# Chenxu1103/UNET-

Measured on AMD Instinct MI355X. Metric: frames/sec 512x512 3-class UNet++ inference; mask vs CPU reference, higher is better.
Workload: dtype f16 (MFMA operands split hi+lo, 3 MFMAs per product, f32 accumulate); 1 GPU; UNet++ 3-class 512x512 batch=16/GPU fp16-MFMA on 1 MI355X, synthetic frames, f32 NCHW in HBM -> uint8 mask in HBM; arch=nested, precision=exact, frames_per_gpu=16, global_batch=16, micro_batch=16, parallelism=frame-sharded x1, weights replicated (RCCL bcast)

## Files before the change

### unet-_amd/csrc/conv3x3_mfma.h

```cpp
#pragma once
#include <hip/hip_runtime.h>
#include <stdint.h>

namespace unetpp {

typedef _Float16 half_t;
typedef __attribute__((ext_vector_type(8))) _Float16 half8;
typedef __attribute__((ext_vector_type(2))) _Float16 half2v;
typedef __attribute__((ext_vector_type(16))) float float16v;
typedef __attribute__((ext_vector_type(4))) unsigned int u32x4;

struct ConvArgs {
  const half_t* in0;
  const half_t* in1;
  const half_t* wpk;
  const float* scale;
  const float* bias;
  half_t* out;
  half_t* pool_out;
  int N, H, W, C0, C1, Cout;
  int tiles_x, tiles_y;
  int nct;
  int nchunks;
  int ksplit;
  float* kpart;
  unsigned* kcnt;
  int gdec[5];
  int pair9;
  const float* head_w;
  const float* head_b;
  int head_C;
  float* logits;
  uint8_t* mask;
  uint8_t* cable;
  uint8_t* tape;
  float* probs;
  int rule;
  float t_cable, t_tape, bg_margin, ct_margin;
  unsigned* status;
  const float* zinit;
  const void* raw_in;
  int raw_fmt;
  const half_t* c1w;
  const float* c1_scale;
  const float* c1_bias;
#ifdef UNETPP_WS_DBG
  int dbg;
  unsigned long long* stamps;
#endif
};

constexpr unsigned ST_OVERFLOW = 1u, ST_NAN = 2u;
constexpr float F16_MAX = 65504.0f;
__device__ __forceinline__ void range_flag(unsigned* status, bool out_of_range, bool is_nan) {
  const unsigned long long bn = __builtin_amdgcn_ballot_w64(is_nan);
  const unsigned long long bo = __builtin_amdgcn_ballot_w64(out_of_range && !is_nan);
  if ((threadIdx.x & 63) == 0 && status) atomicOr(status, (bn ? ST_NAN : 0u) | (bo ? ST_OVERFLOW : 0u));
}

__device__ __forceinline__ void apply_rule(int rule, float p0, float p1, float p2, float tc, float tt, float bgm,
                                           float ctm, bool& cable, bool& tape) {
  const int winner = (p1 > p0) ? ((p2 > p1) ? 2 : 1) : ((p2 > p0) ? 2 : 0);
  if (rule == 1) {
    cable = winner == 1 && p1 >= tc && (p1 - p0) >= bgm;
    tape = winner == 2 && p2 >= tt && (p2 - p0) >= bgm;
  } else if (rule == 2) {
    cable = winner == 1 && p1 >= tc && p0 <= bgm;
    tape = winner == 2 && p2 >= tt && p0 <= bgm;
  } else {
    const bool cand_c = p1 >= tc && p1 >= p0 + bgm;
    const bool cand_t = p2 >= tt && p2 >= p0 + bgm;
    cable = cand_c && p1 >= p2 + ctm;
    tape = cand_t && p2 >= p1 + ctm;
    if (cable && tape) { cable = p1 >= p2; tape = !cable; }
  }
}

template <int P, int KC, int NW, int MW, int WAVES, bool UPF = false>
struct ConvCfg {
  static constexpr int NT = WAVES * 64;
  static constexpr int TH = WAVES * MW, TW = 32, HALO_W = TW + 2, NHALO = (TH + 2) * HALO_W;
  static constexpr int KG = KC / 8, BN = 32 * NW;
  static constexpr int U = P * KG;
  static constexpr int PPP = 64 / U;
  static constexpr int HALO_PIECES = (NHALO + PPP - 1) / PPP;
  static constexpr int HALO_BYTES = HALO_PIECES * 1024;
  static constexpr int HALO_ITERS = (HALO_PIECES + WAVES - 1) / WAVES;
  static constexpr int SLAB_BYTES = P * 9 * KC * BN * 2;
  static constexpr int BUF_BYTES = HALO_BYTES + SLAB_BYTES;
  static constexpr int LSH = TH / 2 + 2, LSW = TW / 2 + 2, LS_PX = LSH * LSW;
  static constexpr int LS_REC = P * 32;
  static constexpr int LS_PIECES = (LS_PX * LS_REC + 1023) / 1024;
  static constexpr int LS_BYTES = UPF ? LS_PIECES * 1024 : 0;
  static constexpr int LS_ITERS = (LS_PIECES + WAVES - 1) / WAVES;
  static constexpr int LDS_BYTES = 2 * BUF_BYTES + 2 * LS_BYTES;
  static constexpr int SLAB_PIECES = SLAB_BYTES / 1024;
  static_assert(U == 2 || U == 4, "unit count per pixel");
  static_assert(SLAB_BYTES % 1024 == 0, "slab must be a whole number of 1 KiB DMA pieces");
  static_assert(LDS_BYTES <= 160 * 1024, "LDS budget");
};

__device__ __forceinline__ void split_f16(float v, half_t& hi, half_t& lo) {
  v = fminf(v, F16_MAX);
  hi = (half_t)v;
  lo = (half_t)(v - (float)hi);
}

typedef __attribute__((address_space(3))) char lds_char_t;

template <class Args>
__device__ __forceinline__ void touch_kernarg_lines() {
  const int* ka = (const int*)__builtin_amdgcn_kernarg_segment_ptr();
  int touched = 0;
#pragma unroll
  for (int o = 0; o < (int)(sizeof(Args) / 4); o += 16) touched |= ka[o];
  asm volatile("" :: "s"(touched));
}

__device__ __forceinline__ void glds16(const void* sbase, unsigned voff, unsigned lds_dst) {
  unsigned keep;
  asm volatile("s_mov_b32 %0, m0\n\ts_mov_b32 m0, %3\n\ts_nop 0\n\tglobal_load_lds_dwordx4 %1, %2\n\ts_mov_b32 m0, %0"
               : "=&s"(keep)
               : "v"(voff), "s"(sbase), "s"(lds_dst)
               : "memory");
}

template <bool NT = false>
__device__ __forceinline__ void blds16(__amdgpu_buffer_rsrc_t rsrc, unsigned voff, int soff, unsigned lds_dst) {
  unsigned keep;
  if (NT)
    asm volatile("s_mov_b32 %0, m0\n\ts_mov_b32 m0, %4\n\ts_nop 0\n\tbuffer_load_dwordx4 %1, %2, %3 offen nt lds\n\ts_mov_b32 m0, %0"
                 : "=&s"(keep)
                 : "v"(voff), "s"(rsrc), "s"(soff), "s"(lds_dst)
                 : "memory");
  else
    asm volatile("s_mov_b32 %0, m0\n\ts_mov_b32 m0, %4\n\ts_nop 0\n\tbuffer_load_dwordx4 %1, %2, %3 offen lds\n\ts_mov_b32 m0, %0"
                 : "=&s"(keep)
                 : "v"(voff), "s"(rsrc), "s"(soff), "s"(lds_dst)
                 : "memory");
}

__device__ __forceinline__ void split_pack2(float v0, float v1, unsigned& wh, unsigned& wl) {
  half2v ph = {(half_t)v0, (half_t)v1};
  wh = __builtin_bit_cast(unsigned, ph);
  unsigned l;
  asm("v_fma_mixlo_f16 %0, %1, -1.0, %2 op_sel_hi:[1,0,0]" : "=v"(l) : "v"(wh), "v"(v0));
  asm("v_fma_mixhi_f16 %0, %1, -1.0, %2 op_sel:[1,0,0] op_sel_hi:[1,0,0]" : "+v"(l) : "v"(wh), "v"(v1));
  wl = l;
}

typedef __attribute__((ext_vector_type(2))) short short2v;
constexpr float X8_LO_DIV = 0.00390625f, X8_X_DIV = 8.0f;
constexpr float X8_LO_MUL = 0.00390625f;
constexpr int X8_SCALE_W = 127 + 6, X8_SCALE_A = 127 - 8;
__device__ __forceinline__ void split_pack4_x8(float v0, float v1, float v2, float v3, unsigned& h0, unsigned& h1, unsigned& l8, unsigned& x8) {
  half2v p0 = {(half_t)v0, (half_t)v1}, p1 = {(half_t)v2, (half_t)v3};
  h0 = __builtin_bit_cast(unsigned, p0); h1 = __builtin_bit_cast(unsigned, p1);
  float l0, l1, l2, l3;
  asm("v_fma_mix_f32 %0, %1, -1.0, %2 op_sel_hi:[1,0,0]" : "=v"(l0) : "v"(h0), "v"(v0));
  asm("v_fma_mix_f32 %0, %1, -1.0, %2 op_sel:[1,0,0] op_sel_hi:[1,0,0]" : "=v"(l1) : "v"(h0), "v"(v1));
  asm("v_fma_mix_f32 %0, %1, -1.0, %2 op_sel_hi:[1,0,0]" : "=v"(l2) : "v"(h1), "v"(v2));
  asm("v_fma_mix_f32 %0, %1, -1.0, %2 op_sel:[1,0,0] op_sel_hi:[1,0,0]" : "=v"(l3) : "v"(h1), "v"(v3));
  short2v t = {0, 0};
  t = __builtin_amdgcn_cvt_scalef32_pk_bf8_f32(t, l0, l1, X8_LO_DIV, false);
  t = __builtin_amdgcn_cvt_scalef32_pk_bf8_f32(t, l2, l3, X8_LO_DIV, true);
  l8 = __builtin_bit_cast(unsigned, t);
  short2v u = {0, 0};
  u = __builtin_amdgcn_cvt_scalef32_pk_bf8_f32(u, v0, v1, X8_X_DIV, false);
  u = __builtin_amdgcn_cvt_scalef32_pk_bf8_f32(u, v2, v3, X8_X_DIV, true);
  x8 = __builtin_bit_cast(unsigned, u);
}

template <int P, bool X8 = false>
__device__ __forceinline__ void pack_store_octets(const float (&v)[16], half_t* dst, size_t blk_stride, bool ok, int h) {
  unsigned wh[4][2], wl[4][2];
  if (X8) {
#pragma unroll
    for (int q = 0; q < 4; ++q) split_pack4_x8(v[4 * q], v[4 * q + 1], v[4 * q + 2], v[4 * q + 3], wh[q][0], wh[q][1], wl[q][0], wl[q][1]);
  }
#pragma unroll
  for (int q = 0; q < 4; ++q)
#pragma unroll
    for (int w2 = 0; w2 < 2; ++w2) {
      const float v0 = v[4 * q + 2 * w2], v1 = v[4 * q + 2 * w2 + 1];
      if (X8) {
      } else if (P == 2) {
        split_pack2(v0, v1, wh[q][w2], wl[q][w2]);
      } else {
        half2v ph = {(half_t)v0, (half_t)v1};
        wh[q][w2] = __builtin_bit_cast(unsigned, ph);
      }
    }
#pragma unroll
  for (int pi = 0; pi < 2; ++pi) {
#pragma unroll
    for (int w2 = 0; w2 < 2; ++w2) {
      auto r = __builtin_amdgcn_permlane32_swap(wh[2 * pi][w2], wh[2 * pi + 1][w2], false, false);
      wh[2 * pi][w2] = r[0]; wh[2 * pi + 1][w2] = r[1];
      if (P == 2) {
        auto r2 = __builtin_amdgcn_permlane32_swap(wl[2 * pi][w2], wl[2 * pi + 1][w2], false, false);
        wl[2 * pi][w2] = r2[0]; wl[2 * pi + 1][w2] = r2[1];
      }
    }
    if (ok) {
      u32x4 o = {wh[2 * pi][0], wh[2 * pi][1], wh[2 * pi + 1][0], wh[2 * pi + 1][1]};
      *(u32x4*)(dst + pi * blk_stride + 8 * h) = o;
      if (P == 2) {
        u32x4 o2 = {wl[2 * pi][0], wl[2 * pi][1], wl[2 * pi + 1][0], wl[2 * pi + 1][1]};
        *(u32x4*)(dst + pi * blk_stride + 16 + 8 * h) = o2;
      }
    }
  }
}

template <int P, bool X8 = false>
__device__ __forceinline__ void pack_store_rows8(const float (&v)[16], half_t* dst, size_t blk_stride, bool ok, int h, bool dbg_nostore = false, bool dbg_coalesced = false) {
#pragma unroll
  for (int pi = 0; pi < 2; ++pi) {
    unsigned wh[4], wl[4];
    if (X8) {
      split_pack4_x8(v[8 * pi], v[8 * pi + 1], v[8 * pi + 2], v[8 * pi + 3], wh[0], wh[1], wl[0], wl[1]);
      split_pack4_x8(v[8 * pi + 4], v[8 * pi + 5], v[8 * pi + 6], v[8 * pi + 7], wh[2], wh[3], wl[2], wl[3]);
    }
#pragma unroll
    for (int i = 0; i < 4; ++i) {
      if (X8) {
      } else if (P == 2) {
        split_pack2(v[8 * pi + 2 * i], v[8 * pi + 2 * i + 1], wh[i], wl[i]);
      } else {
        half2v ph = {(half_t)v[8 * pi + 2 * i], (half_t)v[8 * pi + 2 * i + 1]};
        wh[i] = __builtin_bit_cast(unsigned, ph);
      }
    }
#ifdef UNETPP_WS_DBG
    if (dbg_nostore) {
      asm volatile("" :: "v"(wh[0]), "v"(wh[1]), "v"(wh[2]), "v"(wh[3]));
      if (P == 2) asm volatile("" :: "v"(wl[0]), "v"(wl[1]), "v"(wl[2]), "v"(wl[3]));
      continue;
    }
    if (dbg_coalesced) {
      const int lane_ = (int)(threadIdx.x & 63), p_ = lane_ & 31;
      half_t* row = dst - p_ * (P * 16) + pi * blk_stride;
      if (ok) {
        *(u32x4*)(row + lane_ * 8) = (u32x4){wh[0], wh[1], wh[2], wh[3]};
        if (P == 2) *(u32x4*)(row + 512 + lane_ * 8) = (u32x4){wl[0], wl[1], wl[2], wl[3]};
      }
      continue;
    }
#endif
    if (ok) {
      *(u32x4*)(dst + pi * blk_stride + 8 * h) = (u32x4){wh[0], wh[1], wh[2], wh[3]};
      if (P == 2) *(u32x4*)(dst + pi * blk_stride + 16 + 8 * h) = (u32x4){wl[0], wl[1], wl[2], wl[3]};
    }
  }
}

constexpr int HEAD_FUSED_MAX_CLASSES = 8;

template <int P, int KC, int NW, int MW, int WAVES, bool POOL, bool HEAD = false, bool UPF = false>
__global__ __launch_bounds__(WAVES * 64, 1)
void conv3x3_bias_relu_kernel(ConvArgs a) {
  touch_kernarg_lines<ConvArgs>();
  using C = ConvCfg<P, KC, NW, MW, WAVES, UPF>;
  static_assert(!UPF || (!POOL && !HEAD && KC == 16 && MW == 2), "fused upsample: plain 16-row tiles only");
  constexpr int NT = C::NT, TH = C::TH, TW = C::TW, HALO_W = C::HALO_W;
  constexpr int KG = C::KG, BN = C::BN, PPP = C::PPP;
  constexpr int ITERS = C::HALO_ITERS;
  extern __shared__ __attribute__((aligned(16))) char smem[];

  const int tid = threadIdx.x;
  const int lane = tid & 63;
  const int wave = __builtin_amdgcn_readfirstlane(tid >> 6);
  const int H = a.H, W = a.W;
  const int tiles_img = a.tiles_x * a.tiles_y;
  const int total_tiles = a.N * tiles_img * a.nct;
  const int nch0 = (a.C0 + KC - 1) / KC;
  const unsigned lds_base = (unsigned)(unsigned long)(lds_char_t*)smem;

  const int my_u = lane / PPP;
  const int my_pl = my_u / KG, my_k8 = (my_u % KG) * 8;
  int hyx[ITERS];
#pragma unroll
  for (int it = 0; it < ITERS; ++it) {
    const int hp = (wave + it * WAVES) * PPP + lane % PPP;
    const int hy = hp / HALO_W, hx = hp - hy * HALO_W;
    hyx[it] = (hp < C::NHALO) ? ((hy << 8) | hx) : -1;
  }

  constexpr unsigned OOB = 0x80000000u;
  unsigned voff0[ITERS], voff1[ITERS];
  __amdgpu_buffer_rsrc_t rsrc0, rsrc1;
  const char* wsrc;
  const unsigned img_bytes0 = (unsigned)(H * W * P * a.C0 * 2);
  const unsigned img_bytes1 = (unsigned)((UPF ? (H >> 1) * (W >> 1) : H * W) * P * a.C1 * 2);
  int cur_n, cur_y0, cur_x0, cur_ct;
  auto decode = [&](int t, int& n, int& y0, int& x0, int& ct) {
    ct = t % a.nct;
    int pt = t / a.nct;
    const int tx = pt % a.tiles_x; pt /= a.tiles_x;
    const int ty = pt % a.tiles_y;
    n = pt / a.tiles_y;
    x0 = tx * TW; y0 = ty * TH;
  };
  const int cb0 = a.C0 < 16 ? a.C0 : 16;
  const unsigned plane_bytes0 = (unsigned)(H * W * P * cb0 * 2);
  const int Hs = UPF ? (H >> 1) : H, Ws = UPF ? (W >> 1) : W;
  const unsigned plane_bytes1 = (unsigned)(Hs * Ws * P * 16 * 2);
  constexpr int UP_ITEMS = C::NHALO * KG;
  constexpr int UP_ROUNDS = UPF ? (UP_ITEMS + NT - 1) / NT : 0;
  constexpr int LSR = UPF ? C::LS_ITERS : 1, UPR = UPF ? UP_ROUNDS : 1;
  unsigned voffL[LSR];
  int up_o00[UPR], up_o01[UPR], up_o10[UPR];
  float up_lx1[UPR], up_ly0[UPR], up_ly1[UPR];
  int up_dst[UPR];
  const float up_sh = Hs > 1 ? (float)(Hs - 1) / (float)(H - 1) : 0.f;
  const float up_sw = Ws > 1 ? (float)(Ws - 1) / (float)(W - 1) : 0.f;
  if (UPF) {
#pragma unroll
    for (int r = 0; r < UPR; ++r) {
      const int i = tid + r * NT;
      const int kg = i / C::NHALO, hp = i - kg * C::NHALO;
      up_dst[r] = i < UP_ITEMS ? (hp / PPP) * 1024 + (kg * PPP + hp % PPP) * 16 : -1;
    }
  }
  auto setup_sources = [&](int n, int y0, int x0, int ct) {
#pragma unroll
    for (int it = 0; it < ITERS; ++it) {
      const int hy = hyx[it] >> 8, hx = hyx[it] & 255;
      const int gy = y0 + hy - 1, gx = x0 + hx - 1;
      const int pl = my_pl, k8 = my_k8;
      const bool ok = hyx[it] >= 0 && gy >= 0 && gy < H && gx >= 0 && gx < W;
      const unsigned pix = (unsigned)((gy * W + gx) * P + pl);
      voff0[it] = (ok && k8 < a.C0) ? (unsigned)(k8 >> 4) * plane_bytes0 + (pix * cb0 + (k8 & 15)) * 2u : OOB;
      voff1[it] = ok ? (unsigned)(k8 >> 4) * plane_bytes1 + (pix * 16 + (k8 & 15)) * 2u : OOB;
    }
    rsrc0 = __builtin_amdgcn_make_buffer_rsrc((void*)(a.in0 + (size_t)n * H * W * P * a.C0), 0, (int)img_bytes0, 0x00020000);
    rsrc1 = __builtin_amdgcn_make_buffer_rsrc((void*)(a.in1 ? a.in1 + (size_t)n * Hs * Ws * P * a.C1 : a.in0), 0,
                                              (int)(a.in1 ? img_bytes1 : 0u), 0x00020000);
    wsrc = (const char*)a.wpk + (size_t)ct * a.nchunks * C::SLAB_BYTES;
    if (UPF) {
      const int ybase = (int)(up_sh * (float)max(y0 - 1, 0)), xbase = (int)(up_sw * (float)max(x0 - 1, 0));
      constexpr int PXP = 1024 / C::LS_REC, PARTS = C::LS_REC / 16;
#pragma unroll
      for (int it = 0; it < LSR; ++it) {
        const int lp = (wave + it * WAVES) * PXP + lane / PARTS;
        const int ly = lp / C::LSW, lx = lp - ly * C::LSW;
        const int yy = min(ybase + ly, Hs - 1), xx = min(xbase + lx, Ws - 1);
        voffL[it] = lp < C::LS_PX ? (unsigned)((yy * Ws + xx) * C::LS_REC + (lane % PARTS) * 16) : OOB;
      }
#pragma unroll
      for (int r = 0; r < UPR; ++r) {
        const int i = tid + r * NT;
        const int kg = i / C::NHALO, hp = i - kg * C::NHALO;
        const int hy = hp / HALO_W, hx = hp - hy * HALO_W;
        const int gy = y0 + hy - 1, gx = x0 + hx - 1;
        const bool inside = i < UP_ITEMS && gy >= 0 && gy < H && gx >= 0 && gx < W;
        const float fy = up_sh * (float)max(gy, 0), fx = up_sw * (float)max(gx, 0);
        const int yy0 = min((int)fy, Hs - 1), xx0 = min((int)fx, Ws - 1);
        const int yy1 = yy0 + (yy0 < Hs - 1 ? 1 : 0), xx1 = xx0 + (xx0 < Ws - 1 ? 1 : 0);
        const float ly1 = fminf(fmaxf(fmaf(up_sh, (float)max(gy, 0), -(float)yy0), 0.f), 1.f);
        const float lx1 = fminf(fmaxf(fmaf(up_sw, (float)max(gx, 0), -(float)xx0), 0.f), 1.f);
        const int ry0 = min(max(yy0 - ybase, 0), C::LSH - 1), ry1 = min(max(yy1 - ybase, 0), C::LSH - 1);
        const int rx0 = min(max(xx0 - xbase, 0), C::LSW - 1), rx1 = min(max(xx1 - xbase, 0), C::LSW - 1);
        up_o00[r] = (ry0 * C::LSW + rx0) * C::LS_REC + kg * 16;
        up_o01[r] = (ry0 * C::LSW + rx1) * C::LS_REC + kg * 16;
        up_o10[r] = (ry1 * C::LSW + rx0) * C::LS_REC + kg * 16;
        up_lx1[r] = lx1;
        up_ly0[r] = inside ? 1.f - ly1 : 0.f;
        up_ly1[r] = inside ? ly1 : 0.f;
      }
    }
  };

  auto halo_dma_one = [&](int c, int halo_off, int it) {
    const int piece = wave + it * WAVES;
    if (C::HALO_PIECES % WAVES != 0 && piece >= C::HALO_PIECES) return;
    const unsigned dst = lds_base + halo_off + piece * 1024;
    if (c < nch0) blds16(rsrc0, voff0[it], c * (KC / 16) * (int)plane_bytes0, dst);
    else if (!UPF) blds16(rsrc1, voff1[it], (c - nch0) * (KC / 16) * (int)plane_bytes1, dst);
  };
  const int ls_base = 2 * C::BUF_BYTES;
  auto ls_dma_one = [&](int c, int it) {
    const int piece = wave + it * WAVES;
    if (C::LS_PIECES % WAVES != 0 && piece >= C::LS_PIECES) return;
    blds16(rsrc1, voffL[it], (c - nch0) * (int)plane_bytes1, lds_base + ls_base + (c & 1) * C::LS_BYTES + piece * 1024);
  };
  auto up_item = [&](int c, int halo_off, int r) {
    if (up_dst[r] < 0) return;
    const char* ls = smem + ls_base + (c & 1) * C::LS_BYTES;
    const int o11 = up_o10[r] + (up_o01[r] - up_o00[r]);
    const half8 h00 = *(const half8*)(ls + up_o00[r]), h01 = *(const half8*)(ls + up_o01[r]);
    const half8 h10 = *(const half8*)(ls + up_o10[r]), h11 = *(const half8*)(ls + o11);
    half8 l00, l01, l10, l11;
    if (P == 2) {
      l00 = *(const half8*)(ls + up_o00[r] + 32); l01 = *(const half8*)(ls + up_o01[r] + 32);
      l10 = *(const half8*)(ls + up_o10[r] + 32); l11 = *(const half8*)(ls + o11 + 32);
    }
    const float lx1 = up_lx1[r], lx0 = 1.f - lx1, ly0 = up_ly0[r], ly1 = up_ly1[r];
    half8 oh, ol;
#pragma unroll
    for (int e = 0; e < 8; ++e) {
      float t0, t1;
      if (P == 2) {
        t0 = fmaf(lx1, (float)l01[e], fmaf(lx1, (float)h01[e], fmaf(lx0, (float)l00[e], lx0 * (float)h00[e])));
        t1 = fmaf(lx1, (float)l11[e], fmaf(lx1, (float)h11[e], fmaf(lx0, (float)l10[e], lx0 * (float)h10[e])));
      } else {
        t0 = fmaf(lx1, (float)h01[e], lx0 * (float)h00[e]);
        t1 = fmaf(lx1, (float)h11[e], lx0 * (float)h10[e]);
      }
      const float v = fmaf(ly1, t1, ly0 * t0);
      const half_t hi = (half_t)v;
      oh[e] = hi;
      if (P == 2) ol[e] = (half_t)(v - (float)hi);
    }
    char* dst = smem + halo_off + up_dst[r];
    *(half8*)dst = oh;
    if (P == 2) *(half8*)(dst + KG * PPP * 16) = ol;
  };
  constexpr int DMA_PER_WAVE = (C::SLAB_PIECES + WAVES - 1) / WAVES;
  auto slab_dma_one = [&](int c, int slab_off, int p) {
    const int piece = wave + p * WAVES;
    if (C::SLAB_PIECES % WAVES == 0 || piece < C::SLAB_PIECES)
      glds16(wsrc + (size_t)c * C::SLAB_BYTES + piece * 1024, lane * 16, lds_base + slab_off + piece * 1024);
  };

  int a_off[MW + 2][3];
#pragma unroll
  for (int r = 0; r < MW + 2; ++r)
#pragma unroll
    for (int dx = 0; dx < 3; ++dx) {
      const int hp = (wave * MW + r) * HALO_W + (lane & 31) + dx;
      a_off[r][dx] = (hp / PPP) * 1024 + ((lane >> 5) * PPP + hp % PPP) * 16;
    }
  const int b_lane_off = ((lane >> 5) * BN + (lane & 31)) * 16;

  struct Frag { half8 ah[MW], al[MW], bh[NW], bl[NW]; };
  auto load_frags = [&](Frag& f, const char* halo, const char* slab, int step) {
    const int tap = step % 9, s = step / 9;
    const int dy = tap / 3, dx = tap % 3;
#pragma unroll
    for (int m = 0; m < MW; ++m) {
      const char* p = halo + a_off[m + dy][dx] + (2 * s) * PPP * 16;
// ... 233 lines not shown
```

### unet-_amd/csrc/conv3x3_ws.h

```cpp
#pragma once
#include "conv3x3_mfma.h"

namespace unetpp {

template <int P, bool UPF, bool C0F = false, int NW_ = 1, int MW_ = 4, bool X8_ = false>
struct WsCfg {
  static constexpr bool X8 = X8_;
  static_assert(!X8 || P == 2, "EXACT8 keeps the 64-byte pixel records of the two-plane format");
  static constexpr int NT = 512, NCONS = 4, NPROD = 4, MW = MW_, NW = NW_;
  static constexpr int TH = NCONS * MW, TW = 32, HALO_W = TW + 2, NHALO = (TH + 2) * HALO_W;
  static constexpr int KC = 16, KG = 2, BN = 32 * NW;
  static_assert(MW % 2 == 0 && NW * MW == 4, "108 MFMAs per chunk and consumer wave");
  static constexpr int U = P * KG, PPP = 64 / U;
  static constexpr int HALO_PIECES = (NHALO + PPP - 1) / PPP, HALO_BYTES = HALO_PIECES * 1024;
  static constexpr int HALO_ITERS = (HALO_PIECES + NPROD - 1) / NPROD;
  static constexpr int SLAB_MAIN = 9 * KC * BN * 2;
  static constexpr int SLAB_BYTES = X8 ? SLAB_MAIN + 5 * 2 * 2 * BN * 16 : P * SLAB_MAIN, SLAB_PIECES = SLAB_BYTES / 1024;
  static constexpr int SLAB_ITERS = (SLAB_PIECES + NPROD - 1) / NPROD;
  static constexpr int BUF_BYTES = HALO_BYTES + SLAB_BYTES;
  static constexpr int LSH = TH / 2 + 2, LSW = TW / 2 + 2, LS_PX = LSH * LSW, LS_REC = P * 32;
  static constexpr int LS_PIECES = (LS_PX * LS_REC + 1023) / 1024, LS_BYTES = UPF ? LS_PIECES * 1024 : 0;
  static constexpr int LS_ITERS = (LS_PIECES + NPROD - 1) / NPROD;
  static constexpr int PATCH_H = TH + 4, PATCH_W = TW + 4, PATCH_FLOATS = PATCH_H * PATCH_W * 3;
  static constexpr int PATCH_BYTES = C0F ? ((PATCH_FLOATS * 4 + 64 + 255) / 256) * 256 : 0;
  static constexpr int C0_GROUPS = (NHALO + 15) / 16, C0_ITERS = (C0_GROUPS + NPROD - 1) / NPROD;
  static constexpr bool HANDOFF = !UPF && !C0F;
  static constexpr int STG_WAVE = 2 * 16 * 64 * 4, STG_BYTES = HANDOFF ? NCONS * STG_WAVE : 0;
  static constexpr int LDS_BYTES = 2 * BUF_BYTES + 2 * LS_BYTES + 2 * PATCH_BYTES + STG_BYTES;
  static constexpr int BLK_Y = (TH + 2) / 2, BLK_X = HALO_W / 2, UP_ITEMS = BLK_Y * BLK_X * 4;
  static constexpr int UP_ROUNDS = (UP_ITEMS + NPROD * 64 - 1) / (NPROD * 64);
  static_assert(SLAB_BYTES % 1024 == 0 && LDS_BYTES <= 160 * 1024, "LDS budget");
};

typedef int int4v __attribute__((ext_vector_type(4)));
typedef int int8v __attribute__((ext_vector_type(8)));

__device__ __forceinline__ void lds_barrier() {
  __builtin_amdgcn_fence(__ATOMIC_RELEASE, "workgroup", "local");
  __builtin_amdgcn_s_barrier();
  __builtin_amdgcn_fence(__ATOMIC_ACQUIRE, "workgroup", "local");
}

template <int P, int ROWS, bool POOL, bool HEAD, bool X8 = false>
__device__ __forceinline__ void ws_epilogue(const ConvArgs& a, const float16v (&acc)[ROWS], const float2* sb_lds,
                                            const float* head_lds, int n, int gy0, int x0, int cbase, int lane) {
  const int H = a.H, W = a.W;
  const int h = lane >> 5;
  const int gx = x0 + (lane & 31);
  const int nbo = a.Cout >> 4;
  float v[ROWS][16];
  float vmax = 0.f;
#pragma unroll
  for (int r = 0; r < 16; ++r) {
    const int co = cbase + 16 * (r >> 3) + 8 * h + (r & 7);
    const float2 sb = sb_lds[co];
#pragma unroll
    for (int m = 0; m < ROWS; ++m) {
      v[m][r] = fmaxf(acc[m][r] * sb.x + sb.y, 0.f);
      if (!HEAD) vmax = fmaxf(vmax, v[m][r]);
    }
  }
  if (!HEAD && __builtin_amdgcn_ballot_w64(vmax > F16_MAX)) {
    range_flag(a.status, vmax > F16_MAX, false);
#pragma unroll
    for (int r = 0; r < 16; ++r)
#pragma unroll
      for (int m = 0; m < ROWS; ++m) v[m][r] = fminf(v[m][r], F16_MAX);
  }
  if (!HEAD) {
#pragma unroll
    for (int m = 0; m < ROWS; ++m) {
      const int gy = gy0 + m;
      const bool ok = gy < H && gx < W;
      const size_t blk = (size_t)H * W * P * 16;
      half_t* dst = a.out + ((size_t)n * nbo + (cbase >> 4)) * blk + ((size_t)gy * W + gx) * P * 16;
#ifdef UNETPP_WS_DBG
      pack_store_rows8<P, X8>(v[m], dst, blk, ok, h, (a.dbg & 262144) != 0, (a.dbg & 524288) != 0);
#else
      pack_store_rows8<P, X8>(v[m], dst, blk, ok, h);
#endif
    }
  } else {
    static_assert(!HEAD || ROWS % 2 == 0, "fused head: row pairs");
    const size_t hw = (size_t)H * W;
#pragma unroll
    for (int m2 = 0; m2 < ROWS / 2; ++m2) {
      float lg[HEAD_FUSED_MAX_CLASSES];
#pragma unroll
      for (int c = 0; c < HEAD_FUSED_MAX_CLASSES; ++c) {
        lg[c] = -INFINITY;
        if (c < a.head_C) {
          float wq[16];
#pragma unroll
          for (int q = 0; q < 4; ++q) {
            const float4 w4 = *(const float4*)(head_lds + c * 32 + 16 * (q >> 1) + 8 * h + 4 * (q & 1));
            wq[4 * q] = w4.x; wq[4 * q + 1] = w4.y; wq[4 * q + 2] = w4.z; wq[4 * q + 3] = w4.w;
          }
          const float bc = head_lds[a.head_C * 32 + c];
          float p0 = 0.f, p1 = 0.f;
#pragma unroll
          for (int r = 0; r < 16; ++r) { p0 = fmaf(v[2 * m2][r], wq[r], p0); p1 = fmaf(v[2 * m2 + 1][r], wq[r], p1); }
          auto sw = __builtin_amdgcn_permlane32_swap(__builtin_bit_cast(unsigned, p0), __builtin_bit_cast(unsigned, p1), false, false);
          unsigned s0 = sw[0], s1 = sw[1];
          asm volatile("s_nop 1" : "+v"(s0), "+v"(s1));
          lg[c] = bc + (__builtin_bit_cast(float, s0) + __builtin_bit_cast(float, s1));
        }
      }
      const int gy = gy0 + 2 * m2 + h;
      const bool ok = gy < H && gx < W;
      const size_t pix = (size_t)gy * W + gx;
      float best = lg[0];
      int besti = 0;
#pragma unroll
      for (int c = 1; c < HEAD_FUSED_MAX_CLASSES; ++c)
        if (lg[c] > best) { best = lg[c]; besti = c; }
      bool is_cable = besti == 1, is_tape = besti == 2;
      if (a.probs || a.rule) {
        float pe[HEAD_FUSED_MAX_CLASSES], sum = 0.f;
#pragma unroll
        for (int c = 0; c < HEAD_FUSED_MAX_CLASSES; ++c) {
          pe[c] = (c < a.head_C) ? expf(lg[c] - best) : 0.f;
          sum += pe[c];
        }
#pragma unroll
        for (int c = 0; c < HEAD_FUSED_MAX_CLASSES; ++c) {
          pe[c] = pe[c] / sum;
          if (ok && a.probs && c < a.head_C) a.probs[((size_t)n * a.head_C + c) * hw + pix] = pe[c];
        }
        if (a.rule) apply_rule(a.rule, pe[0], pe[1], pe[2], a.t_cable, a.t_tape, a.bg_margin, a.ct_margin, is_cable, is_tape);
      }
      if (ok) {
        if (a.logits) {
#pragma unroll
          for (int c = 0; c < HEAD_FUSED_MAX_CLASSES; ++c)
            if (c < a.head_C) a.logits[((size_t)n * a.head_C + c) * hw + pix] = lg[c];
        }
        const size_t o = (size_t)n * hw + pix;
        if (a.mask) a.mask[o] = (uint8_t)besti;
        if (a.cable) a.cable[o] = is_cable;
        if (a.tape) a.tape[o] = is_tape;
      }
    }
  }
  if (POOL) {
    static_assert(!POOL || ROWS % 2 == 0, "fused pool: row pairs");
    const int Hp = H >> 1, Wp = W >> 1;
#pragma unroll
    for (int m2 = 0; m2 < ROWS / 2; ++m2) {
      float pv[16];
#pragma unroll
      for (int r = 0; r < 16; ++r) {
        const float vm = fmaxf(v[2 * m2][r], v[2 * m2 + 1][r]);
        const float vn = __builtin_bit_cast(float, __builtin_amdgcn_mov_dpp(__builtin_bit_cast(int, vm), 0xB1, 0xF, 0xF, true));
        pv[r] = fmaxf(vm, vn);
      }
      const int py = (gy0 >> 1) + m2, px = (x0 >> 1) + ((lane & 31) >> 1);
      const bool ok = ((lane & 1) == 0) && py < Hp && px < Wp;
      const size_t blk = (size_t)Hp * Wp * P * 16;
      half_t* dst = a.pool_out + ((size_t)n * nbo + (cbase >> 4)) * blk + ((size_t)py * Wp + px) * P * 16;
#ifdef UNETPP_WS_DBG
      pack_store_rows8<P, X8>(pv, dst, blk, ok, h, (a.dbg & 262144) != 0);
#else
      pack_store_rows8<P, X8>(pv, dst, blk, ok, h);
#endif
    }
  }
}

template <int P, bool POOL, bool HEAD, bool UPF, bool C0F = false, int NW = 1, int MWP = 4, bool X8 = false, bool CAT2 = false>
__global__ __launch_bounds__(512, 2) void conv3x3_ws_kernel(ConvArgs a) {
  using C = WsCfg<P, UPF, C0F, NW, MWP, X8>;
  static_assert(!C0F || (!UPF && !HEAD && P == 2 && NW == 1), "fused first block: exact mode, no other fusion in the loader");
  static_assert(!HEAD || NW == 1, "the fused head needs all 32 channels of x0_4 in one 32-block");
  constexpr int NT = C::NT, MW = C::MW, TH = C::TH, TW = C::TW, HALO_W = C::HALO_W;
  constexpr int KC = C::KC, KG = C::KG, BN = C::BN, PPP = C::PPP;
  static_assert(!(POOL && HEAD) && !(UPF && (POOL || HEAD)), "one fused extra per kernel");
  static_assert(!CAT2 || (!UPF && !C0F && !POOL && !HEAD), "two full-resolution sources: the plain kernel only");
  extern __shared__ __attribute__((aligned(16))) char smem[];
#ifdef UNETPP_WS_DBG
  const unsigned long long rt_entry = __builtin_amdgcn_s_memrealtime();
#endif
  touch_kernarg_lines<ConvArgs>();

  const int tid = threadIdx.x;
  const int lane = tid & 63;
  const int wave = __builtin_amdgcn_readfirstlane(tid >> 6);
  const int H = a.H, W = a.W;
  const int tiles_img = a.tiles_x * a.tiles_y;
  const int KS = a.ksplit;
  const int total_tiles = a.N * tiles_img * a.nct * KS;
  const int nch0 = (a.C0 + KC - 1) / KC;
  const unsigned lds_base = (unsigned)(unsigned long)(lds_char_t*)smem;

  float2* sb_lds = (float2*)(smem + C::LDS_BYTES);
  float* head_lds = (float*)(smem + C::LDS_BYTES + a.Cout * 8);
  if (wave < C::NCONS) {
    for (int i = tid; i < a.Cout; i += C::NCONS * 64) sb_lds[i] = make_float2(a.scale[i], a.bias[i]);
    if (HEAD) {
      for (int i = tid; i < a.head_C * 32; i += C::NCONS * 64) head_lds[i] = a.head_w[i];
      for (int i = tid; i < a.head_C; i += C::NCONS * 64) head_lds[a.head_C * 32 + i] = a.head_b[i];
    }
  }

#ifdef UNETPP_WS_DBG
  const unsigned long long rt_staged = __builtin_amdgcn_s_memrealtime();
#endif
  const int G = (int)gridDim.x;
  const int slot = (G % 8 == 0) ? ((int)blockIdx.x % 8) * (G / 8) + (int)blockIdx.x / 8 : (int)blockIdx.x;
  int dec_ks = 0, dec_ct = 0, dec_tx = 0, dec_ty = 0, dec_n = 0, dec_t = -1;
  const int g_ks = a.gdec[0], g_ct = a.gdec[1], g_tx = a.gdec[2], g_ty = a.gdec[3], g_n = a.gdec[4];
  const bool small_radix = total_tiles < (1 << 22);
  auto divmod = [&](const int u, const int d, int& q, int& r) {
    int qq, rr;
    if (small_radix) {
      qq = (int)((float)u * __builtin_amdgcn_rcpf((float)d));
      rr = u - qq * d;
      const int up = rr >= d ? 1 : 0, dn = rr < 0 ? 1 : 0;
      qq += up - dn; rr += (dn - up) * d;
    } else {
      qq = u / d; rr = u - qq * d;
    }
    q = qq; r = rr;
  };
  auto decode = [&](int t, int& n, int& y0, int& x0) {
    if (t != dec_t) {
      if (dec_t >= 0 && t == dec_t + G) {
        dec_ks += g_ks;
        int carry = dec_ks >= KS ? 1 : 0;
        dec_ks -= carry ? KS : 0;
        dec_ct += g_ct + carry;
        carry = dec_ct >= a.nct ? 1 : 0;
        dec_ct -= carry ? a.nct : 0;
        dec_tx += g_tx + carry;
        carry = dec_tx >= a.tiles_x ? 1 : 0;
        dec_tx -= carry ? a.tiles_x : 0;
        dec_ty += g_ty + carry;
        carry = dec_ty >= a.tiles_y ? 1 : 0;
        dec_ty -= carry ? a.tiles_y : 0;
        dec_n += g_n + carry;
      } else {
        int u = t;
        divmod(u, KS, u, dec_ks);
        divmod(u, a.nct, u, dec_ct);
        divmod(u, a.tiles_x, u, dec_tx);
        divmod(u, a.tiles_y, dec_n, dec_ty);
      }
      dec_t = t;
    }
    n = dec_n; x0 = dec_tx * TW; y0 = dec_ty * TH;
  };
  if (slot >= total_tiles) return;
  const bool handoff = C::HANDOFF && a.nchunks >= 2 && KS == 1;

  typedef __attribute__((ext_vector_type(4))) float float4v;
  const int plane_id = tid - C::NCONS * 64;
  constexpr int PATCH_ELEMS = C::PATCH_FLOATS, PATCH_LOADS = C0F ? (PATCH_ELEMS + C::NPROD * 64 - 1) / (C::NPROD * 64) : 1;
  const int patch_base = 2 * C::BUF_BYTES + 2 * C::LS_BYTES;
  int pe_rc[PATCH_LOADS], pe_idx[PATCH_LOADS];
  if (C0F) {
#pragma unroll
    for (int i = 0; i < PATCH_LOADS; ++i) {
      const int e = plane_id + i * (C::NPROD * 64);
      int row, col, cs, idx;
      if (a.raw_fmt == 0) {
        const int ch = e / (C::PATCH_H * C::PATCH_W), rem = e - ch * (C::PATCH_H * C::PATCH_W);
        row = rem / C::PATCH_W; col = rem - row * C::PATCH_W; cs = ch; idx = rem * 3 + ch;
      } else {
        row = e / (C::PATCH_W * 3); const int b = e - row * (C::PATCH_W * 3);
        col = b / 3; cs = b - col * 3; idx = (row * C::PATCH_W + col) * 3 + (2 - cs);
      }
      pe_rc[i] = (row << 16) | (col << 2) | cs;
      pe_idx[i] = (e < PATCH_ELEMS && plane_id >= 0) ? idx : -1;
    }
  }
  auto patch_fetch = [&](int n, int y0, int x0, float (&val)[PATCH_LOADS]) {
    const size_t img = (size_t)H * W * 3;
    const __amdgpu_buffer_rsrc_t rs = __builtin_amdgcn_make_buffer_rsrc(
        (void*)((const char*)a.raw_in + (size_t)n * img * (a.raw_fmt == 0 ? 4 : 1)), 0, (int)(img * (a.raw_fmt == 0 ? 4 : 1)), 0x00020000);
    bool beyond = false;
#pragma unroll
    for (int i = 0; i < PATCH_LOADS; ++i) {
      const int gy = y0 - 2 + (pe_rc[i] >> 16), gx = x0 - 2 + ((pe_rc[i] >> 2) & 0x3fff), cs = pe_rc[i] & 3;
      const bool ok = pe_idx[i] >= 0 && gy >= 0 && gy < H && gx >= 0 && gx < W;
      float v;
      if (a.raw_fmt == 0) {
        v = __builtin_bit_cast(float, __builtin_amdgcn_raw_buffer_load_b32(rs, ok ? ((cs * H + gy) * W + gx) * 4 : (int)0x80000000, 0, 0));
      } else {
        const unsigned char b8 = __builtin_amdgcn_raw_buffer_load_b8(rs, ok ? (gy * W + gx) * 3 + cs : (int)0x80000000, 0, 0);
        v = __fdiv_rn((float)b8, 255.0f);
      }
      beyond |= !(fabsf(v) <= F16_MAX);
      val[i] = v;
    }
    if (__builtin_amdgcn_ballot_w64(beyond)) {
      bool nan = false;
#pragma unroll
      for (int i = 0; i < PATCH_LOADS; ++i) { nan |= val[i] != val[i]; val[i] = __builtin_amdgcn_fmed3f(val[i], -F16_MAX, F16_MAX); }
      range_flag(a.status, beyond, nan);
    }
  };
  auto patch_store = [&](int buf, const float (&val)[PATCH_LOADS]) {
    unsigned* pd = (unsigned*)(smem + patch_base + buf * C::PATCH_BYTES);
#pragma unroll
    for (int i = 0; i < PATCH_LOADS; ++i)
      if (pe_idx[i] >= 0) {
        unsigned wh, wl;
        split_pack2(val[i], 0.f, wh, wl);
        pd[pe_idx[i]] = (wh & 0xffffu) | (wl << 16);
      }
  };
  if (C0F && wave >= C::NCONS) {
    constexpr int SL_IT = (2 * C::SLAB_PIECES + C::NPROD - 1) / C::NPROD;
#pragma unroll
    for (int it = 0; it < SL_IT; ++it) {
      const int piece = (wave - C::NCONS) + it * C::NPROD;
      if (piece < 2 * C::SLAB_PIECES) {
        const int c = piece / C::SLAB_PIECES, pc = piece - c * C::SLAB_PIECES;
        glds16((const char*)a.wpk + (size_t)c * C::SLAB_BYTES + pc * 1024, lane * 16,
               lds_base + c * C::BUF_BYTES + C::HALO_BYTES + pc * 1024);
      }
    }
    if (plane_id < 32) {
      *(float*)(smem + patch_base + PATCH_ELEMS * 4 + (plane_id & 15) * 4 + (plane_id >> 4) * C::PATCH_BYTES) = 0.f;
    }
    int n0, y00, x00;
    decode(slot, n0, y00, x00);
    float pv[PATCH_LOADS];
    patch_fetch(n0, y00, x00, pv);
    patch_store(0, pv);
    asm volatile("s_waitcnt vmcnt(0)" ::: "memory");
  }
  if (C0F) __syncthreads();

#ifdef UNETPP_WS_DBG
#define WS_STAMP(i) { const unsigned long long now_ = __builtin_readcyclecounter(); st_sum[i] += now_ - st_t; st_t = now_; \
                      if (ev_ptr && ev_ptr < ev_end) *ev_ptr++ = ((unsigned long long)(i) << 56) | __builtin_amdgcn_s_memrealtime(); }
#define WS_EVLOG(role) unsigned long long* ev_ptr = (a.stamps && (a.dbg & 131072) && lane == 0 && blockIdx.x < 1024) ? a.stamps + (size_t)1024 * 32 + ((size_t)blockIdx.x * 2 + (role)) * 64 : nullptr; \
                       unsigned long long* const ev_end = ev_ptr + 60; if (ev_ptr) *ev_ptr++ = (63ull << 56) | rt_entry;
#define WS_STAMP_IN(i) if (a.dbg & 32768) { __builtin_amdgcn_sched_barrier(0); asm volatile("s_waitcnt lgkmcnt(0)" ::: "memory"); WS_STAMP(i) __builtin_amdgcn_sched_barrier(0); }
#define WS_EVT(i) { if (ev_ptr && ev_ptr < ev_end) *ev_ptr++ = ((unsigned long long)(i) << 56) | __builtin_amdgcn_s_memrealtime(); }
#else
#define WS_STAMP(i) {}
#define WS_STAMP_IN(i) {}
#define WS_EVT(i) {}
#endif
  if (C0F && wave >= C::NCONS) {
    const int pw = wave - C::NCONS;
#ifdef UNETPP_WS_DBG
    unsigned long long st_sum[11] = {0, 0, 0, 0, 0, 0, 0, 0, 0, 0, 0};
    unsigned long long st_t = __builtin_readcyclecounter();
    WS_EVLOG(1)
    if (pw != 0) ev_ptr = nullptr;
#endif
#ifndef UNETPP_C0_PRIO
#define UNETPP_C0_PRIO 1
#endif
    if (UNETPP_C0_PRIO) __builtin_amdgcn_s_setprio(UNETPP_C0_PRIO);
    typedef __attribute__((ext_vector_type(4))) float f32x4;
    typedef __attribute__((ext_vector_type(2))) unsigned u32x2;
    const int pxl = lane & 15, kq = lane >> 4;
    half8 wa_h[2], wa_l[2];
#pragma unroll
    for (int c = 0; c < 2; ++c) {
      wa_h[c] = *(const half8*)(a.c1w + ((size_t)(c * 2 + 0) * 64 + lane) * 8);
      wa_l[c] = *(const half8*)(a.c1w + ((size_t)(c * 2 + 1) * 64 + lane) * 8);
    }
    float sc1[2][4], bi1[2][4];
#pragma unroll
    for (int c = 0; c < 2; ++c)
#pragma unroll
      for (int r = 0; r < 4; ++r) { sc1[c][r] = a.c1_scale[16 * c + 4 * kq + r]; bi1[c][r] = a.c1_bias[16 * c + 4 * kq + r]; }
    int koff[8];
#pragma unroll
    for (int i = 0; i < 8; ++i) {
      if (kq < 3) koff[i] = (kq * C::PATCH_W * 3 + i) * 4;
      else koff[i] = i < 3 ? (i * C::PATCH_W * 3 + 8) * 4 : -1;
    }
    int g = 0;
    for (int tile = slot; tile < total_tiles; tile += G) {
      int n, y0, x0;
      decode(tile, n, y0, x0);
      const int tbuf = (g >> 1) & 1;
      const char* patch = smem + patch_base + tbuf * C::PATCH_BYTES;
      const int zero_off = PATCH_ELEMS * 4;
#pragma unroll
      for (int c = 0; c < 2; ++c, ++g) {
        float pv[PATCH_LOADS];
        const int ntile = tile + G;
        const bool have_next = c == 0 && ntile < total_tiles;
        if (have_next) {
          int n2, y2, x2;
          decode(ntile, n2, y2, x2);
          patch_fetch(n2, y2, x2, pv);
        }
        WS_STAMP(0)
        char* himg = smem + c * C::BUF_BYTES;
        float vmax = 0.f;
#ifndef UNETPP_C0_GB
#define UNETPP_C0_GB 2
#endif
        constexpr int GB = UNETPP_C0_GB;
        static_assert(C::C0_ITERS % GB == 0, "group batches");
        const int dst_lane = ((kq >> 1) * PPP + pxl) * 16 + (kq & 1) * 8;
        auto groups = [&](auto interior_tag) {
          constexpr bool INTERIOR = decltype(interior_tag)::value;
          int hy = (pw * 16 + pxl) / HALO_W, hx = (pw * 16 + pxl) - hy * HALO_W;
#pragma nounroll
          for (int b0 = 0; b0 < C::C0_ITERS; b0 += GB) {
            unsigned bw[GB][8];
            int ghy[GB], ghx[GB];
#pragma unroll
            for (int k = 0; k < GB; ++k) {
              ghy[k] = hy; ghx[k] = hx;
              const int hyc = min(hy, TH + 1);
              const int pix_off = (hyc * C::PATCH_W + hx) * 12;
#pragma unroll
              for (int i = 0; i < 8; ++i) bw[k][i] = *(const unsigned*)(patch + (koff[i] >= 0 ? pix_off + koff[i] : zero_off + 4 * i));
              hy += 1; hx += 64 - HALO_W;
              if (hx >= HALO_W) { hx -= HALO_W; hy += 1; }
            }
            f32x4 acc[GB];
#pragma unroll
            for (int k = 0; k < GB; ++k) {
              unsigned bh[4], bl[4];
#pragma unroll
              for (int i = 0; i < 4; ++i) {
                bh[i] = __builtin_amdgcn_perm(bw[k][2 * i + 1], bw[k][2 * i], 0x05040100u);
                bl[i] = __builtin_amdgcn_perm(bw[k][2 * i + 1], bw[k][2 * i], 0x07060302u);
              }
              const half8 xh = __builtin_bit_cast(half8, (u32x4){bh[0], bh[1], bh[2], bh[3]});
              const half8 xl = __builtin_bit_cast(half8, (u32x4){bl[0], bl[1], bl[2], bl[3]});
              acc[k] = (f32x4){0.f, 0.f, 0.f, 0.f};
              acc[k] = __builtin_amdgcn_mfma_f32_16x16x32_f16(wa_h[c], xl, acc[k], 0, 0, 0);
              acc[k] = __builtin_amdgcn_mfma_f32_16x16x32_f16(wa_l[c], xh, acc[k], 0, 0, 0);
              acc[k] = __builtin_amdgcn_mfma_f32_16x16x32_f16(wa_h[c], xh, acc[k], 0, 0, 0);
            }
#pragma unroll
            for (int k = 0; k < GB; ++k) {
              const int gi = pw + (b0 + k) * C::NPROD;
              const bool valid = gi * 16 + pxl < C::NHALO;
              float v[4];
#pragma unroll
              for (int r = 0; r < 4; ++r) v[r] = acc[k][r] * sc1[c][r] + bi1[c][r];
              vmax = fmaxf(fmaxf(vmax, v[0]), v[1]); vmax = fmaxf(fmaxf(vmax, v[2]), v[3]);
#pragma unroll
              for (int r = 0; r < 4; ++r) v[r] = __builtin_amdgcn_fmed3f(v[r], 0.f, F16_MAX);
              if (!INTERIOR) {
                const int gy = y0 - 1 + ghy[k], gx = x0 - 1 + ghx[k];
                const bool inside = gy >= 0 && gy < H && gx >= 0 && gx < W;
#pragma unroll
                for (int r = 0; r < 4; ++r) v[r] = inside ? v[r] : 0.f;
              }
              unsigned oh0, oh1, ol0, ol1;
              if (X8) {
                split_pack4_x8(v[0], v[1], v[2], v[3], oh0, oh1, ol0, ol1);
              } else {
                split_pack2(v[0], v[1], oh0, ol0);
                split_pack2(v[2], v[3], oh1, ol1);
              }
              if (valid) {
                char* dst = himg + gi * 1024 + dst_lane;
                *(u32x2*)dst = (u32x2){oh0, oh1};
                *(u32x2*)(dst + KG * PPP * 16) = (u32x2){ol0, ol1};
              }
            }
          }
        };
        if (y0 >= 1 && y0 + TH < H && x0 >= 1 && x0 + TW < W) groups(std::true_type());
        else groups(std::false_type());
        if (__builtin_amdgcn_ballot_w64(vmax > F16_MAX)) range_flag(a.status, vmax > F16_MAX, false);
        WS_STAMP(1)
        if (have_next) patch_store(tbuf ^ 1, pv);
        WS_STAMP(2)
        lds_barrier();
        WS_STAMP(3)
      }
    }
#ifdef UNETPP_WS_DBG
    if (a.stamps && pw == 0 && lane == 0)
#pragma unroll
      for (int i = 0; i < 11; ++i) a.stamps[((size_t)blockIdx.x * 2 + 1) * 16 + i] = st_sum[i];
    if (a.stamps && pw == 0 && lane == 0) a.stamps[((size_t)blockIdx.x * 2 + 1) * 16 + 12] = __builtin_amdgcn_s_memrealtime();
#endif
    return;
  }

  if (wave >= C::NCONS) {
    const int pw = wave - C::NCONS;
#ifdef UNETPP_WS_DBG
    const unsigned long long rt_prod = __builtin_amdgcn_s_memrealtime();
    { const int pr = (a.dbg >> 10) & 3; if (pr == 1) __builtin_amdgcn_s_setprio(1); else if (pr == 2) __builtin_amdgcn_s_setprio(2); else if (pr == 3) __builtin_amdgcn_s_setprio(3); }
#endif
    constexpr unsigned OOB = 0x80000000u;
    constexpr int ITERS = C::HALO_ITERS;
    int my_u = lane / PPP;
#ifdef UNETPP_WS_DBG
    if (a.dbg & 16384) my_u = lane % C::U;
#endif
    const int my_pl = my_u / KG, my_k8 = (my_u % KG) * 8;
    int hyx[ITERS];
#pragma unroll
    for (int it = 0; it < ITERS; ++it) {
      int hp = (pw + it * C::NPROD) * PPP + lane % PPP;
#ifdef UNETPP_WS_DBG
      if (a.dbg & 16384) hp = (pw + it * C::NPROD) * PPP + lane / C::U;
#endif
      const int hy = hp / HALO_W, hx = hp - hy * HALO_W;
      hyx[it] = (hp < C::NHALO) ? ((hy << 8) | hx) : -1;
    }
    const int cb0 = a.C0 < 16 ? a.C0 : 16;
    const unsigned plane_bytes0 = (unsigned)H * (unsigned)W * (unsigned)(P * cb0 * 2);
    const unsigned img_bytes0 = (unsigned)H * (unsigned)W * (unsigned)(P * a.C0 * 2);
    const int Hs = H >> 1, Ws = W >> 1;
    const unsigned plane_bytes1 = (unsigned)Hs * (unsigned)Ws * (unsigned)(P * 16 * 2);
    const unsigned img_bytes1 = (unsigned)Hs * (unsigned)Ws * (unsigned)(P * a.C1 * 2);
    const float up_sh = Hs > 1 ? (float)(Hs - 1) / (float)(H - 1) : 0.f;
    const float up_sw = Ws > 1 ? (float)(Ws - 1) / (float)(W - 1) : 0.f;

    int lane_off0[ITERS];
#pragma unroll
    for (int it = 0; it < ITERS; ++it) {
      const int hy = hyx[it] >> 8, hx = hyx[it] & 255;
      const bool valid = hyx[it] >= 0 && my_k8 < a.C0;
      lane_off0[it] = valid ? (my_k8 >> 4) * (int)plane_bytes0 + ((((hy - 1) * W + (hx - 1)) * P + my_pl) * cb0 + (my_k8 & 15)) * 2 : (int)OOB;
    }
    unsigned voff0[ITERS];
    __amdgpu_buffer_rsrc_t rsrc0, rsrc1;
    constexpr int LSR = UPF ? C::LS_ITERS : 1, UPR = UPF ? C::UP_ROUNDS : 1;
    unsigned voffL[LSR];
    int up_o00[UPR], up_o01[UPR], up_o10[UPR];
    float up_wx[UPR][4], up_wy[UPR][4];
    int up_st[UPR][4];
    int rd_swap = (P == 2 && !X8 && (lane & 16)) ? 32 : 0;
#ifdef UNETPP_WS_DBG
    if (a.dbg & 32) rd_swap = 0;
#endif
    if (UPF) {
#pragma unroll
      for (int r = 0; r < UPR; ++r) {
        const int i = pw * 64 + lane + r * (C::NPROD * 64);
        const int q = i & 3, blk = i >> 2;
        const int by = blk / C::BLK_X, bx = blk - by * C::BLK_X;
        const int hp0 = (2 * by) * HALO_W + 2 * bx;
#pragma unroll
        for (int px = 0; px < 4; ++px) {
          const int hp = hp0 + (px >> 1) * HALO_W + ((px & 1) ^ ((q >> 1) & 1));
          up_st[r][px] = (hp / PPP) * 1024 + ((q >> 1) * PPP + hp % PPP) * 16 + (q & 1) * 8;
        }
        if (i >= C::UP_ITEMS) up_st[r][0] = -1;
      }
    }

    auto setup_tile = [&](int n, int y0, int x0) {
      if (y0 >= 1 && y0 + TH < H && x0 >= 1 && x0 + TW < W) {
        const unsigned origin = ((unsigned)y0 * (unsigned)W + (unsigned)x0) * (unsigned)(P * cb0 * 2);
#pragma unroll
        for (int it = 0; it < ITERS; ++it) voff0[it] = origin + (unsigned)lane_off0[it];
      } else {
#pragma unroll
        for (int it = 0; it < ITERS; ++it) {
          const int hy = hyx[it] >> 8, hx = hyx[it] & 255;
          const int gy = y0 + hy - 1, gx = x0 + hx - 1;
          const bool ok = hyx[it] >= 0 && gy >= 0 && gy < H && gx >= 0 && gx < W;
          const unsigned pix = (unsigned)((gy * W + gx) * P + my_pl);
          voff0[it] = (ok && my_k8 < a.C0) ? (unsigned)(my_k8 >> 4) * plane_bytes0 + (pix * cb0 + (my_k8 & 15)) * 2u : OOB;
        }
      }
      rsrc0 = __builtin_amdgcn_make_buffer_rsrc((void*)(a.in0 + (size_t)n * H * W * P * a.C0), 0, (int)img_bytes0, 0x00020000);
      if (CAT2)
        rsrc1 = __builtin_amdgcn_make_buffer_rsrc((void*)(a.in1 + (size_t)n * H * W * P * a.C1), 0, (int)((unsigned)H * (unsigned)W * (unsigned)(P * a.C1 * 2)), 0x00020000);
      if (UPF) {
        rsrc1 = __builtin_amdgcn_make_buffer_rsrc((void*)(a.in1 + (size_t)n * Hs * Ws * P * a.C1), 0, (int)img_bytes1, 0x00020000);
        const int ybase = (int)(up_sh * (float)max(y0 - 1, 0)), xbase = (int)(up_sw * (float)max(x0 - 1, 0));
        constexpr int PXP = 1024 / C::LS_REC, PARTS = C::LS_REC / 16;
#pragma unroll
        for (int it = 0; it < LSR; ++it) {
          const int lp = (pw + it * C::NPROD) * PXP + lane / PARTS;
          const int ly = lp / C::LSW, lx = lp - ly * C::LSW;
          const int yy = min(ybase + ly, Hs - 1), xx = min(xbase + lx, Ws - 1);
          voffL[it] = lp < C::LS_PX ? (unsigned)((yy * Ws + xx) * C::LS_REC + (lane % PARTS) * 16) : OOB;
        }
#pragma unroll
        for (int r = 0; r < UPR; ++r) {
          const int i = pw * 64 + lane + r * (C::NPROD * 64);
          const int q = i & 3, blk = i >> 2;
          const int by = blk / C::BLK_X, bx = blk - by * C::BLK_X;
          const int gyA = y0 + 2 * by - 1, gxA = x0 + 2 * bx - 1;
          const int gyR = (gyA + 1 < H) ? gyA + 1 : gyA, gxR = (gxA + 1 < W) ? gxA + 1 : gxA;
          const float fyR = up_sh * (float)max(gyR, 0), fxR = up_sw * (float)max(gxR, 0);
          const int yy0 = min((int)fyR, Hs - 1), xx0 = min((int)fxR, Ws - 1);
          const int yy1 = yy0 + (yy0 < Hs - 1 ? 1 : 0), xx1 = xx0 + (xx0 < Ws - 1 ? 1 : 0);
          const int ry0 = min(max(yy0 - ybase, 0), C::LSH - 1), ry1 = min(max(yy1 - ybase, 0), C::LSH - 1);
          const int rx0 = min(max(xx0 - xbase, 0), C::LSW - 1), rx1 = min(max(xx1 - xbase, 0), C::LSW - 1);
          up_o00[r] = (ry0 * C::LSW + rx0) * C::LS_REC + q * 8 + rd_swap;
          up_o01[r] = (ry0 * C::LSW + rx1) * C::LS_REC + q * 8 + rd_swap;
          up_o10[r] = (ry1 * C::LSW + rx0) * C::LS_REC + q * 8 + rd_swap;
          const int xs = (q >> 1) & 1;
#pragma unroll
          for (int k = 0; k < 2; ++k) {
            const int gy = gyA + k, gx = gxA + (k ^ xs);
            const bool iny = gy >= 0 && gy < H, inx = gx >= 0 && gx < W;
            const float ly1 = fminf(fmaxf(up_sh * (float)max(gy, 0) - (float)yy0, 0.f), 1.f);
            const float lx1 = fminf(fmaxf(up_sw * (float)max(gx, 0) - (float)xx0, 0.f), 1.f);
            up_wy[r][2 * k] = iny ? 1.f - ly1 : 0.f; up_wy[r][2 * k + 1] = iny ? ly1 : 0.f;
            up_wx[r][2 * k] = inx ? 1.f - lx1 : 0.f; up_wx[r][2 * k + 1] = inx ? lx1 : 0.f;
          }
        }
      }
    };

#ifdef UNETPP_WS_DBG
    unsigned long long st_sum[11] = {0, 0, 0, 0, 0, 0, 0, 0, 0, 0, 0};
    unsigned long long st_t = 0;
    WS_EVLOG(1)
    if (pw != 0) ev_ptr = nullptr;
    if (ev_ptr) { *ev_ptr++ = (48ull << 56) | rt_staged; *ev_ptr++ = (49ull << 56) | rt_prod; }
    WS_EVT(50)
#endif
    auto up_rounds = [&](int c, int halo_off) {
      typedef __attribute__((ext_vector_type(2))) unsigned u32x2;
      const char* ls = smem + 2 * C::BUF_BYTES + (c & 1) * C::LS_BYTES;
      u32x2 hq[UPR][4], lq[UPR][4];
#pragma unroll
      for (int r = 0; r < UPR; ++r) {
        const int o11 = up_o10[r] + (up_o01[r] - up_o00[r]);
        const int off[4] = {up_o00[r], up_o01[r], up_o10[r], o11};
#pragma unroll
        for (int k = 0; k < 4; ++k) {
#ifdef UNETPP_WS_DBG
          if (a.dbg & 512) { hq[r][k] = (u32x2){0x3c003c00u, 0x3c003c00u}; lq[r][k] = (u32x2){0u, 0u}; continue; }
#endif
          hq[r][k] = *(const u32x2*)(ls + off[k]);
          if (P == 2) lq[r][k] = *(const u32x2*)(ls + (off[k] ^ 32));
        }
      }
      __builtin_amdgcn_sched_barrier(0);
      WS_STAMP_IN(8)
#pragma unroll
      for (int r = 0; r < UPR; ++r) {
        float v[4][4];
#pragma unroll
        for (int e = 0; e < 4; ++e) {
          float cc[4];
#pragma unroll
          for (int k = 0; k < 4; ++k) {
            if (X8) {
              const unsigned lo16 = __builtin_bit_cast(unsigned, (e >> 1) ? __builtin_amdgcn_cvt_scalef32_pk_f16_bf8(lq[r][k][0], X8_LO_MUL, true)
                                                                        : __builtin_amdgcn_cvt_scalef32_pk_f16_bf8(lq[r][k][0], X8_LO_MUL, false));
              if (e & 1) asm("v_fma_mix_f32 %0, %1, 1.0, %2 op_sel:[1,0,1] op_sel_hi:[1,0,1]" : "=v"(cc[k]) : "v"(hq[r][k][e >> 1]), "v"(lo16));
              else asm("v_fma_mix_f32 %0, %1, 1.0, %2 op_sel_hi:[1,0,1]" : "=v"(cc[k]) : "v"(hq[r][k][e >> 1]), "v"(lo16));
            } else if (P == 2) {
              if (e & 1) asm("v_fma_mix_f32 %0, %1, 1.0, %2 op_sel:[1,0,1] op_sel_hi:[1,0,1]" : "=v"(cc[k]) : "v"(hq[r][k][e >> 1]), "v"(lq[r][k][e >> 1]));
              else asm("v_fma_mix_f32 %0, %1, 1.0, %2 op_sel_hi:[1,0,1]" : "=v"(cc[k]) : "v"(hq[r][k][e >> 1]), "v"(lq[r][k][e >> 1]));
            } else {
              const unsigned hw = hq[r][k][e >> 1];
              const half2v hv = __builtin_bit_cast(half2v, hw);
              cc[k] = (float)hv[e & 1];
            }
          }
#pragma unroll
          for (int kx = 0; kx < 2; ++kx) {
            const float t0 = fmaf(up_wx[r][2 * kx + 1], cc[1], up_wx[r][2 * kx] * cc[0]);
            const float t1 = fmaf(up_wx[r][2 * kx + 1], cc[3], up_wx[r][2 * kx] * cc[2]);
#pragma unroll
            for (int ky = 0; ky < 2; ++ky) v[2 * ky + kx][e] = fmaf(up_wy[r][2 * ky + 1], t1, up_wy[r][2 * ky] * t0);
          }
        }
        WS_STAMP_IN(9)
#ifdef UNETPP_WS_DBG
        if (a.dbg & 64) { if (v[0][0] == 12345.f && v[3][3] == 7.f && v[1][2] == 3.f && v[2][1] == 9.f) a.status[1] = 1; continue; }
#endif
        if (up_st[r][0] >= 0) {
#pragma unroll
          for (int ky = 0; ky < 2; ++ky)
#pragma unroll
            for (int kx = 0; kx < 2; ++kx) {
              const int px = 2 * ky + kx;
              unsigned h0, h1, l0 = 0, l1 = 0;
              if (X8) {
                split_pack4_x8(v[px][0], v[px][1], v[px][2], v[px][3], h0, h1, l0, l1);
              } else if (P == 2) {
                split_pack2(v[px][0], v[px][1], h0, l0);
                split_pack2(v[px][2], v[px][3], h1, l1);
              } else {
                half2v a0 = {(half_t)v[px][0], (half_t)v[px][1]}, a1 = {(half_t)v[px][2], (half_t)v[px][3]};
                h0 = __builtin_bit_cast(unsigned, a0); h1 = __builtin_bit_cast(unsigned, a1);
              }
              const u32x2 oh = {h0, h1}, ol = {l0, l1};
              char* dst = smem + halo_off + up_st[r][px];
              *(u32x2*)dst = oh;
              if (P == 2) *(u32x2*)(dst + KG * PPP * 16) = ol;
            }
        }
        WS_STAMP_IN(10)
      }
    };

    const int stg_base = 2 * C::BUF_BYTES + 2 * C::LS_BYTES + 2 * C::PATCH_BYTES;
    int hn = 0, hy0 = 0, hx0 = 0, hct = 0;
    bool have_handoff = false;
    auto handoff_epilogue = [&]() {
      const char* st = smem + stg_base + pw * C::STG_WAVE + lane * 16;
      float16v pair[2];
#pragma unroll
      for (int i = 0; i < 2; ++i)
#pragma unroll
        for (int q = 0; q < 4; ++q) {
          typedef __attribute__((ext_vector_type(4))) float f32x4;
          const f32x4 v4 = *(const f32x4*)(st + (i * 4 + q) * 1024);
          pair[i][4 * q] = v4[0]; pair[i][4 * q + 1] = v4[1]; pair[i][4 * q + 2] = v4[2]; pair[i][4 * q + 3] = v4[3];
        }
      const int gy0 = hy0 + pw * MW + (MW == 4 ? 2 : 0);
      const int cbase = hct * BN + (MW == 4 ? 0 : 32);
      ws_epilogue<P, 2, POOL, HEAD, X8>(a, pair, sb_lds, head_lds, hn, gy0, hx0, cbase, lane);
    };
    int g = 0;
    const bool slabs_stay = a.nchunks == 2 && a.nct == 1 && KS == 1;
    const int chunks_per_share = KS == 1 ? a.nchunks : a.nchunks / KS;
#ifdef UNETPP_WS_DBG
    st_t = __builtin_readcyclecounter();
#endif
    WS_EVT(51)
    for (int tile = slot; tile < total_tiles; tile += G) {
      int n, y0, x0;
      decode(tile, n, y0, x0);
      WS_EVT(52)
      const char* wsrc = (const char*)a.wpk + (size_t)dec_ct * a.nchunks * C::SLAB_BYTES;
      const int tile_ct = dec_ct;
      const int c_begin = dec_ks * chunks_per_share, c_end = c_begin + chunks_per_share;
      setup_tile(n, y0, x0);
      WS_STAMP(7)
      for (int c = c_begin; c < c_end; ++c, ++g) {
        const int buf = (g & 1) * C::BUF_BYTES;
#ifdef UNETPP_WS_DBG
        if (!(a.dbg & 2))
#endif
        if (c < nch0) {
#pragma unroll
          for (int it = 0; it < ITERS; ++it) {
            const int piece = pw + it * C::NPROD;
            if (C::HALO_PIECES % C::NPROD == 0 || piece < C::HALO_PIECES)
              blds16<true>(rsrc0, voff0[it], c * (int)plane_bytes0, lds_base + buf + piece * 1024);
          }
        } else if (CAT2) {
#pragma unroll
          for (int it = 0; it < ITERS; ++it) {
            const int piece = pw + it * C::NPROD;
            if (C::HALO_PIECES % C::NPROD == 0 || piece < C::HALO_PIECES)
              blds16<true>(rsrc1, voff0[it], (c - nch0) * (int)plane_bytes0, lds_base + buf + piece * 1024);
          }
        }
#ifdef UNETPP_WS_DBG
        if (!(a.dbg & 8))
#endif
        if (!(slabs_stay && g >= 2))
#pragma unroll
        for (int it = 0; it < C::SLAB_ITERS; ++it) {
          const int piece = pw + it * C::NPROD;
          if (C::SLAB_PIECES % C::NPROD == 0 || piece < C::SLAB_PIECES)
            glds16(wsrc + (size_t)c * C::SLAB_BYTES + piece * 1024, lane * 16, lds_base + buf + C::HALO_BYTES + piece * 1024);
        }
        if (!UPF) { WS_STAMP(0) }
        if (UPF) {
#ifdef UNETPP_WS_DBG
          if (!(a.dbg & 2))
#endif
          if (c + 1 < a.nchunks && c + 1 >= nch0) {
#pragma unroll
            for (int it = 0; it < LSR; ++it) {
              const int piece = pw + it * C::NPROD;
              if (C::LS_PIECES % C::NPROD == 0 || piece < C::LS_PIECES)
                blds16(rsrc1, voffL[it], (c + 1 - nch0) * (int)plane_bytes1,
                       lds_base + 2 * C::BUF_BYTES + ((c + 1) & 1) * C::LS_BYTES + piece * 1024);
            }
          }
          if (c >= nch0) { WS_STAMP(3) } else { WS_STAMP(0) }
#ifdef UNETPP_WS_DBG
          if (!(a.dbg & 1))
#endif
          if (c >= nch0) up_rounds(c, buf);
          if (c >= nch0) { WS_STAMP(4) } else { WS_STAMP(0) }
        }
#ifdef UNETPP_WS_DBG
        if (!(a.dbg & 128))
#endif
        if (handoff && c == 1 && have_handoff) handoff_epilogue();
        asm volatile("s_waitcnt vmcnt(0)" ::: "memory");
        if (UPF && c >= nch0) { WS_STAMP(5) } else { WS_STAMP(1) }
        lds_barrier();
        if (UPF && c >= nch0) { WS_STAMP(6) } else { WS_STAMP(2) }
      }
      hn = n; hy0 = y0; hx0 = x0; hct = tile_ct; have_handoff = true;
    }
    if (handoff) {
      lds_barrier();
      if (have_handoff) handoff_epilogue();
    }
#ifdef UNETPP_WS_DBG
    if (a.stamps && pw == 0 && lane == 0)
#pragma unroll
      for (int i = 0; i < 11; ++i) a.stamps[((size_t)blockIdx.x * 2 + 1) * 16 + i] = st_sum[i];
    if (a.stamps && pw == 0 && lane == 0) a.stamps[((size_t)blockIdx.x * 2 + 1) * 16 + 12] = __builtin_amdgcn_s_memrealtime();
#endif
    return;
  }

  const int cw = wave;
#ifdef UNETPP_WS_DBG
  { const int pr = (a.dbg >> 12) & 3; if (pr == 1) __builtin_amdgcn_s_setprio(1); else if (pr == 2) __builtin_amdgcn_s_setprio(2); else if (pr == 3) __builtin_amdgcn_s_setprio(3); }
#endif
  int a_off[MW + 2][3];
#pragma unroll
  for (int r = 0; r < MW + 2; ++r)
#pragma unroll
    for (int dx = 0; dx < 3; ++dx) {
      const int hp = (cw * MW + r) * HALO_W + (lane & 31) + dx;
      a_off[r][dx] = (hp / PPP) * 1024 + ((lane >> 5) * PPP + hp % PPP) * 16;
    }
  const int b_lane_off = ((lane >> 5) * BN + (lane & 31)) * 16;
  struct AFrag { half8 h[MW + 2], l[MW + 2]; };
  struct BFrag { half8 h[NW], l[NW]; };
  auto load_a = [&](AFrag& f, const char* halo, int dx) {
#pragma unroll
    for (int r = 0; r < MW + 2; ++r) {
      const char* p = halo + a_off[r][dx];
      f.h[r] = *(const half8*)p;
      if (P == 2) f.l[r] = *(const half8*)(p + KG * PPP * 16);
    }
  };
  auto load_a_part = [&](AFrag& f, const char* halo, int dx, int r0, int r1) {
#pragma unroll
    for (int r = 0; r < MW + 2; ++r)
      if (r >= r0 && r < r1) {
        const char* p = halo + a_off[r][dx];
        f.h[r] = *(const half8*)p;
        if (P == 2) f.l[r] = *(const half8*)(p + KG * PPP * 16);
      }
  };
  auto load_b = [&](BFrag& f, const char* slab, int tap) {
#pragma unroll
    for (int j = 0; j < NW; ++j) {
      const int off = b_lane_off + (tap * KG * BN + j * 32) * 16;
      f.h[j] = *(const half8*)(slab + off);
      if (P == 2) f.l[j] = *(const half8*)(slab + off + 9 * KC * BN * 2);
    }
  };
  float16v acc[MW][NW];
  auto run_mfma = [&](const AFrag& fa, const BFrag& fb, int dy) {
#pragma unroll
    for (int m = 0; m < MW; ++m)
#pragma unroll
      for (int j = 0; j < NW; ++j) {
        if (P == 2) {
          acc[m][j] = __builtin_amdgcn_mfma_f32_32x32x16_f16(fb.h[j], fa.l[m + dy], acc[m][j], 0, 0, 0);
          acc[m][j] = __builtin_amdgcn_mfma_f32_32x32x16_f16(fb.l[j], fa.h[m + dy], acc[m][j], 0, 0, 0);
        }
        acc[m][j] = __builtin_amdgcn_mfma_f32_32x32x16_f16(fb.h[j], fa.h[m + dy], acc[m][j], 0, 0, 0);
      }
  };
  auto run_mfma_first = [&](const AFrag& fa, const BFrag& fb) {
    const float16v zero = {0.f, 0.f, 0.f, 0.f, 0.f, 0.f, 0.f, 0.f, 0.f, 0.f, 0.f, 0.f, 0.f, 0.f, 0.f, 0.f};
#pragma unroll
    for (int m = 0; m < MW; ++m)
#pragma unroll
      for (int j = 0; j < NW; ++j) {
        if (P == 2) {
          acc[m][j] = __builtin_amdgcn_mfma_f32_32x32x16_f16(fb.h[j], fa.l[m], zero, 0, 0, 0);
          acc[m][j] = __builtin_amdgcn_mfma_f32_32x32x16_f16(fb.l[j], fa.h[m], acc[m][j], 0, 0, 0);
          acc[m][j] = __builtin_amdgcn_mfma_f32_32x32x16_f16(fb.h[j], fa.h[m], acc[m][j], 0, 0, 0);
        } else {
          acc[m][j] = __builtin_amdgcn_mfma_f32_32x32x16_f16(fb.h[j], fa.h[m], zero, 0, 0, 0);
        }
      }
  };

  int g = 0;
#ifdef UNETPP_WS_DBG
  unsigned long long st_sum[8] = {0, 0, 0, 0, 0, 0, 0, 0};
  unsigned long long st_t = __builtin_readcyclecounter();
  const unsigned long long rt_begin = __builtin_amdgcn_s_memrealtime();
  WS_EVLOG(0)
  if (cw != 0) ev_ptr = nullptr;
  if (ev_ptr) *ev_ptr++ = (62ull << 56) | rt_begin;
#endif
  for (int tile = slot; tile < total_tiles; tile += G) {
    int n, y0, x0;
    decode(tile, n, y0, x0);
    const int ct = dec_ct, ks = dec_ks;
    const int c_begin = ks * (a.nchunks / KS), c_end = c_begin + a.nchunks / KS;
#pragma unroll
    for (int m = 0; m < MW; ++m)
#pragma unroll
      for (int j = 0; j < NW; ++j) {
        if (a.zinit && ks == 0) {
          typedef __attribute__((ext_vector_type(4))) float f32x4;
          const int gy = y0 + cw * MW + m, gx = x0 + (lane & 31);
          const bool in = gy < H && gx < W;
          const float* zp = a.zinit + (((size_t)n * (a.Cout >> 5) + ((ct * BN + j * 32) >> 5)) * ((size_t)H * W) + (size_t)gy * W + gx) * 32 + 8 * (lane >> 5);
#pragma unroll
          for (int q = 0; q < 4; ++q) {
            f32x4 z4 = {0.f, 0.f, 0.f, 0.f};
            if (in) z4 = *(const f32x4*)(zp + 16 * (q >> 1) + 4 * (q & 1));
#pragma unroll
            for (int i = 0; i < 4; ++i) acc[m][j][4 * q + i] = z4[i];
          }
        }
      }
    const bool from_zero = a.zinit == nullptr || ks != 0;
    int4v x9[MW];
    if (X8) {
#pragma unroll
      for (int m = 0; m < MW; ++m) x9[m] = (int4v){0, 0, 0, 0};
    }
    WS_STAMP(3)
    for (int c = c_begin; c < c_end; ++c, ++g) {
      lds_barrier();
      WS_STAMP(0)
      const char* halo = smem + (g & 1) * C::BUF_BYTES;
      const char* slab = halo + C::HALO_BYTES;
#ifdef UNETPP_WS_DBG
      if (a.dbg & 16) continue;
#endif
      if constexpr (X8) {
        constexpr int R = MW + 2;
        const char* xslab = slab + C::SLAB_MAIN;
        struct BM { half8 w[NW]; };
        struct BX { int8v w[NW]; };
        auto load_h = [&](half8 (&f)[R], int dx, int r0, int r1) {
#pragma unroll
          for (int r = 0; r < R; ++r)
            if (r >= r0 && r < r1) f[r] = *(const half8*)(halo + a_off[r][dx]);
        };
        auto load_x = [&](int dxa, int ra, int dxb, int rb) {
          const int4v lo = *(const int4v*)(halo + a_off[ra][dxa] + KG * PPP * 16);
          const int4v hi = *(const int4v*)(halo + a_off[rb][dxb] + KG * PPP * 16);
          return __builtin_shufflevector(lo, hi, 0, 1, 2, 3, 4, 5, 6, 7);
        };
        auto load_bm = [&](BM& f, int tap) {
#pragma unroll
          for (int j = 0; j < NW; ++j) f.w[j] = *(const half8*)(slab + b_lane_off + (tap * KG * BN + j * 32) * 16);
        };
        auto load_bx = [&](BX& f, int pair) {
#pragma unroll
          for (int j = 0; j < NW; ++j) {
            const char* p = xslab + pair * (2 * 2 * BN * 16) + b_lane_off + j * 32 * 16;
            const int4v lo = *(const int4v*)p, hi = *(const int4v*)(p + 2 * BN * 16);
            f.w[j] = __builtin_shufflevector(lo, hi, 0, 1, 2, 3, 4, 5, 6, 7);
          }
        };
        auto main_step = [&](const BM& b, const half8 (&hf)[R], int dy, bool first) {
#ifdef UNETPP_WS_DBG
          if (a.dbg & 4) return;
#endif
          const float16v zero = {0.f, 0.f, 0.f, 0.f, 0.f, 0.f, 0.f, 0.f, 0.f, 0.f, 0.f, 0.f, 0.f, 0.f, 0.f, 0.f};
#pragma unroll
          for (int m = 0; m < MW; ++m)
#pragma unroll
            for (int j = 0; j < NW; ++j)
              acc[m][j] = __builtin_amdgcn_mfma_f32_32x32x16_f16(b.w[j], hf[m + dy], first ? zero : acc[m][j], 0, 0, 0);
        };
        auto cross_step = [&](const BX& b, const int8v (&x)[R], int r0) {
#ifdef UNETPP_WS_DBG
          if (a.dbg & (4 | 65536)) return;
#endif
#pragma unroll
          for (int m = 0; m < MW; ++m)
#pragma unroll
            for (int j = 0; j < NW; ++j)
              acc[m][j] = __builtin_amdgcn_mfma_scale_f32_32x32x64_f8f6f4(b.w[j], x[m + r0], acc[m][j], 0 , 1 ,
                                                                         0, X8_SCALE_W, 0, X8_SCALE_A);
        };
        half8 h0[R], h1[R];
        int8v xa[R];
        BM bm0, bm1;
        BX bx0, bx1;
        load_h(h0, 0, 0, R);
        load_bm(bm0, 0);
        const bool first = c == c_begin && from_zero;
#pragma unroll
        for (int dy = 0; dy < 3; ++dy) {
          BM& b = (dy & 1) ? bm1 : bm0;
          BM& bn = (dy & 1) ? bm0 : bm1;
          load_bm(bn, dy < 2 ? (dy + 1) * 3 : 1);
          load_h(h1, 1, 2 * dy, 2 * dy + 2);
          __builtin_amdgcn_sched_barrier(0);
          if (dy == 0 && first) main_step(b, h0, 0, true); else main_step(b, h0, dy, false);
          __builtin_amdgcn_sched_barrier(0);
        }
#pragma unroll
        for (int dy = 0; dy < 3; ++dy) {
          BM& b = ((3 + dy) & 1) ? bm1 : bm0;
          BM& bn = ((3 + dy) & 1) ? bm0 : bm1;
          if (dy < 2) load_bm(bn, (dy + 1) * 3 + 1); else load_bx(bx0, 0);
#pragma unroll
          for (int r = 2 * dy; r < 2 * dy + 2 && r < R; ++r) xa[r] = load_x(0, r, 1, r);
          __builtin_amdgcn_sched_barrier(0);
          main_step(b, h1, dy, false);
          __builtin_amdgcn_sched_barrier(0);
        }
#pragma unroll
        for (int pr = 0; pr < 3; ++pr) {
          BX& b = (pr & 1) ? bx1 : bx0;
          BX& bn = (pr & 1) ? bx0 : bx1;
          if (pr < 2) load_bx(bn, pr + 1); else load_bm(bm0, 2);
          load_h(h0, 2, 2 * pr, 2 * pr + 2);
          __builtin_amdgcn_sched_barrier(0);
          cross_step(b, xa, pr);
          __builtin_amdgcn_sched_barrier(0);
        }
#pragma unroll
        for (int dy = 0; dy < 3; ++dy) {
          BM& b = (dy & 1) ? bm1 : bm0;
          BM& bn = (dy & 1) ? bm0 : bm1;
          if (dy < 2) load_bm(bn, (dy + 1) * 3 + 2); else load_bx(bx1, 3);
#pragma unroll
          for (int r = 2 * dy; r < 2 * dy + 2 && r < R; ++r) xa[r] = load_x(2, r, 2, r + 1 < R ? r + 1 : r);
          __builtin_amdgcn_sched_barrier(0);
          main_step(b, h0, dy, false);
          __builtin_amdgcn_sched_barrier(0);
        }
        load_bx(bx0, 4);
        int4v cur[MW];
#pragma unroll
        for (int m = 0; m < MW; ++m) cur[m] = *(const int4v*)(halo + a_off[m + 2][2] + KG * PPP * 16);
        __builtin_amdgcn_sched_barrier(0);
        cross_step(bx1, xa, 0);
        __builtin_amdgcn_sched_barrier(0);
        if (!(a.pair9 && ((c - c_begin) & 1) == 0)) {
          int8v xq[R];
#pragma unroll
          for (int m = 0; m < MW; ++m) xq[m] = __builtin_shufflevector(x9[m], cur[m], 0, 1, 2, 3, 4, 5, 6, 7);
          cross_step(bx0, xq, 0);
        }
#pragma unroll
        for (int m = 0; m < MW; ++m) x9[m] = cur[m];
        __builtin_amdgcn_sched_barrier(0);
        WS_STAMP(1)
        continue;
      }
      AFrag fa0, fa1;
      BFrag fb0, fb1;
      load_a(fa0, halo, 0);
      load_b(fb0, slab, 0);
#pragma unroll
      for (int dx = 0; dx < 3; ++dx) {
        AFrag& fa = (dx & 1) ? fa1 : fa0;
        AFrag& fan = (dx & 1) ? fa0 : fa1;
#pragma unroll
        for (int dy = 0; dy < 3; ++dy) {
          const int step = dx * 3 + dy;
          BFrag& fb = (step & 1) ? fb1 : fb0;
          BFrag& fbn = (step & 1) ? fb0 : fb1;
          if (step + 1 < 9) {
            const int ndx = (step + 1) / 3, ndy = (step + 1) % 3;
            load_b(fbn, slab, ndy * 3 + ndx);
          }
          if (dx < 2) load_a_part(fan, halo, dx + 1, 2 * dy, 2 * dy + 2);
          __builtin_amdgcn_sched_barrier(0);
#ifdef UNETPP_WS_DBG
          if (!(a.dbg & 4))
#endif
          {
            if (step == 0 && c == c_begin && from_zero) run_mfma_first(fa, fb);
            else run_mfma(fa, fb, dy);
          }
          __builtin_amdgcn_sched_barrier(0);
        }
      }
      WS_STAMP(1)
    }
#ifdef UNETPP_WS_DBG
    if (a.dbg & 256) { if (acc[0][0][0] == 12345.f && acc[MW - 1][NW - 1][5] == 7.f) a.status[1] = 1; continue; }
#endif
    if (KS > 1) {
      typedef __attribute__((ext_vector_type(4))) float f32x4;
      const int tile_id = tile / KS;
      const int ntile = total_tiles / KS;
      constexpr int WAVE_BYTES = MW * NW * 16 * 64 * 4;
      const __amdgpu_buffer_rsrc_t prs = __builtin_amdgcn_make_buffer_rsrc((void*)a.kpart, 0, KS * ntile * C::NCONS * WAVE_BYTES, 0x00020000);
      const int mine = ((ks * ntile + tile_id) * C::NCONS + cw) * WAVE_BYTES + lane * 16;
#pragma unroll
      for (int m = 0; m < MW; ++m)
#pragma unroll
        for (int j = 0; j < NW; ++j)
#pragma unroll
          for (int q = 0; q < 4; ++q)
            __builtin_amdgcn_raw_buffer_store_b128(__builtin_bit_cast(u32x4, (f32x4){acc[m][j][4 * q], acc[m][j][4 * q + 1], acc[m][j][4 * q + 2], acc[m][j][4 * q + 3]}),
                                                   prs, mine + ((m * NW + j) * 4 + q) * 1024, 0, 16 );
      asm volatile("s_waitcnt vmcnt(0)" ::: "memory");
      unsigned old = 0;
      if (lane == 0) old = __hip_atomic_fetch_add(a.kcnt + tile_id * C::NCONS + cw, 1u, __ATOMIC_RELAXED, __HIP_MEMORY_SCOPE_AGENT);
      old = __builtin_amdgcn_readfirstlane(old);
      if (old != (unsigned)(KS - 1)) { WS_STAMP(2) continue; }
      __builtin_amdgcn_fence(__ATOMIC_ACQUIRE, "wavefront");
      if (lane == 0) __hip_atomic_store(a.kcnt + tile_id * C::NCONS + cw, 0u, __ATOMIC_RELAXED, __HIP_MEMORY_SCOPE_AGENT);
      constexpr int HALF = MW * NW * 2;
      auto fetch = [&](f32x4 (&pv)[HALF], int u) {
        const int src = (((u >> 1) * ntile + tile_id) * C::NCONS + cw) * WAVE_BYTES + lane * 16 + (u & 1) * HALF * 1024;
#pragma unroll
        for (int t = 0; t < HALF; ++t) pv[t] = __builtin_bit_cast(f32x4, __builtin_amdgcn_raw_buffer_load_b128(prs, src + t * 1024, 0, 16 ));
      };
      auto add = [&](const f32x4 (&pv)[HALF], int u) {
#pragma unroll
        for (int m = 0; m < MW; ++m)
#pragma unroll
          for (int j = 0; j < NW; ++j)
#pragma unroll
            for (int q = 0; q < 4; ++q) {
              const int t = (m * NW + j) * 4 + q;
              if ((t >= HALF) != ((u & 1) != 0)) continue;
#pragma unroll
              for (int i = 0; i < 4; ++i) acc[m][j][4 * q + i] = u < 2 ? pv[t % HALF][i] : acc[m][j][4 * q + i] + pv[t % HALF][i];
            }
      };
      f32x4 pa[HALF], pb[HALF];
      fetch(pa, 0);
      for (int u = 0; u < 2 * KS; u += 2) {
        fetch(pb, u + 1);
        add(pa, u);
        if (u + 2 < 2 * KS) fetch(pa, u + 2);
        add(pb, u + 1);
      }
    }
#pragma unroll
    for (int m2 = 0; m2 < MW / 2; ++m2)
#pragma unroll
      for (int j = 0; j < NW; ++j) {
        const bool give = handoff && (MW == 4 ? m2 == 1 : j == 1);
        if (give) {
          char* st = smem + (2 * C::BUF_BYTES + 2 * C::LS_BYTES + 2 * C::PATCH_BYTES) + cw * C::STG_WAVE + lane * 16;
#pragma unroll
          for (int i = 0; i < 2; ++i)
#pragma unroll
            for (int q = 0; q < 4; ++q) {
              typedef __attribute__((ext_vector_type(4))) float f32x4;
              const float16v& v = acc[2 * m2 + i][j];
              *(f32x4*)(st + (i * 4 + q) * 1024) = (f32x4){v[4 * q], v[4 * q + 1], v[4 * q + 2], v[4 * q + 3]};
            }
        } else {
          const float16v pair[2] = {acc[2 * m2][j], acc[2 * m2 + 1][j]};
          ws_epilogue<P, 2, POOL, HEAD, X8>(a, pair, sb_lds, head_lds, n, y0 + cw * MW + 2 * m2, x0, ct * BN + j * 32, lane);
        }
      }
    WS_STAMP(2)
  }
  if (handoff) lds_barrier();
#ifdef UNETPP_WS_DBG
  if (a.stamps && cw == 0 && lane == 0)
#pragma unroll
    for (int i = 0; i < 4; ++i) a.stamps[((size_t)blockIdx.x * 2) * 16 + i] = st_sum[i];
  if (a.stamps && cw == 0 && lane == 0) {
    a.stamps[((size_t)blockIdx.x * 2) * 16 + 4] = rt_begin;
    a.stamps[((size_t)blockIdx.x * 2) * 16 + 6] = rt_entry;
    a.stamps[((size_t)blockIdx.x * 2) * 16 + 5] = __builtin_amdgcn_s_memrealtime();
  }
#endif
}
#undef WS_STAMP

}
```

### unet-_amd/csrc/unetpp_abi.hip

```cpp
#include <hip/hip_runtime.h>

#include <algorithm>
#include <cmath>
#include <cstdarg>
#include <cstdio>
#include <cstdlib>
#include <cstring>
#include <string>
#include <map>
#include <mutex>
#include <set>
#include <tuple>
#include <utility>
#include <vector>

#include "abi_common.h"
#include "aux_kernels.h"
#include "conv3x3_mfma.h"
#include "conv3x3_ws.h"
#include "convt2x2_mfma.h"
#include "tapmm_ws.h"

using namespace unetpp;

namespace {

thread_local std::string g_create_error;

constexpr uint32_t BLOB_MAGIC = 0x50504e55u;
constexpr uint32_t DS_BLOB_MAGIC = 0x53444e55u;
constexpr int BLOB_VERSION = 1;
const int NB[5] = {32, 64, 128, 256, 512};
const int SB[4] = {64, 128, 256, 512};

struct Tensor {
  std::string name;
  size_t off = 0;
  int C = 0;
  int lvl = 0;
  bool virt = false;
};

struct ConvLayer {
  std::string name;
  int cin_real = 0;
  int cout = 0;
  int lvl = 0;
  int in = -1, in2 = -1, out = -1, pool = -1;
  bool do_pool = false;
  int zt = -1;
  int y_t = -1, low_t = -1;
  half_t* tapw = nullptr;
  bool c0f = false;
  bool upf = false;
  bool ws = false;
  size_t w_off = 0, b_off = 0;
  int KC = 16, NW = 1, MW = 2, WAVES = 8;
  int nchunks = 1;
  half_t* wpk = nullptr;
  float* scale = nullptr;
  float* mult = nullptr;
};

struct ConvTLayer {
  std::string name;
  int cin = 0, cout = 0, lvl = 0;
  int in = -1, out = -1;
  size_t w_off = 0, b_off = 0;
  half_t* wpk = nullptr;
  float* scale = nullptr;
  float* mult = nullptr;
};

enum OpKind { OP_CONVERT, OP_CONV, OP_UP, OP_CONVT, OP_HEAD, OP_TAPMM, OP_UPSUM, OP_DS };
struct Op {
  OpKind kind;
  int idx = -1;
  int out = -1;
  bool fuse_head = false;
};

struct ProfRec {
  std::string name;
  double flops = 0, bytes = 0;
  int ev0 = -1, ev1 = -1;
};

}

struct unetpp_engine : unetpp_engine_common {
  int P = 2;
  bool x8 = false;
  int mb = 1;
  int num_cus = 256;
  char* arena = nullptr;
  size_t arena_bytes = 0;
  float* blob = nullptr;
  size_t blob_floats = 0;
  bool weights_loaded = false;
  std::vector<Tensor> tensors;
  std::vector<ConvLayer> convs;
  std::vector<ConvTLayer> convts;
  std::vector<Op> ops;
  int n_blob_layers = 0;
  int t_in8 = -1, t_head_in = -1;
  int head_cx = 32;
  size_t head_w_off = 0, head_b_off = 0;
  bool prof_on = false;
  std::vector<ProfRec> prof;
  int prof_used = 0;
  std::vector<hipEvent_t> evpool;
  int ev_used = 0;
  int prof_prev_ev = -1;
  hipStream_t prof_prev_stream = nullptr;
  int last_b = 0, last_h = 0, last_w = 0;
  bool keep_all = false;
  int nstreams = 1;
  size_t act_bytes = 0;
  size_t last_slot_off = 0;
  hipStream_t streams[4] = {nullptr, nullptr, nullptr, nullptr};
  hipEvent_t ev_start = nullptr, ev_done[4] = {nullptr, nullptr, nullptr, nullptr};
  half_t* c1w = nullptr;
  int c0f_conv1 = -1;
  unsigned* d_status = nullptr;
  int ksplit_max = 16, ksplit_min_chunks = 4, ksplit_gate = 4;
  int t_kpart = -1, t_kcnt = -1;
  bool kcnt_dirty = false;
  float* ds_w = nullptr;
  size_t ds_w_off[4] = {0, 0, 0, 0};
  float* ds_scratch[4] = {nullptr, nullptr, nullptr, nullptr};
  size_t ds_scr_off[4] = {0, 0, 0, 0};
  bool ds_loaded = false;
};

namespace unetpp {

unetpp_engine_common* unetpp_common(unetpp_engine* e) { return e; }

int fail(unetpp_engine* e, int code, const char* fmt, ...) {
  char buf[512];
  va_list ap;
  va_start(ap, fmt);
  vsnprintf(buf, sizeof buf, fmt, ap);
  va_end(ap);
  if (e) e->err = buf; else g_create_error = buf;
  return code;
}

hipError_t allow_full_lds(const void* kernel, int device, int bytes) {
  static std::mutex mu;
  static std::set<std::pair<int, const void*>> done;
  std::lock_guard<std::mutex> lock(mu);
  if (done.count({device, kernel})) return hipSuccess;
  hipError_t st = hipFuncSetAttribute(kernel, hipFuncAttributeMaxDynamicSharedMemorySize, bytes);
  if (st == hipSuccess) done.insert({device, kernel});
  return st;
}

}

namespace {

size_t blob_payload_floats(int arch, int C, int cin, int* n_layers = nullptr) {
  size_t n = 0;
  int layers = 0;
  if (arch == UNETPP_ARCH_NESTED) {
    int ci[9] = {cin, NB[0], NB[1], NB[2], NB[3], NB[3] + NB[4], NB[2] + NB[3], NB[1] + NB[2], NB[0] + NB[1]};
    int co[9] = {NB[0], NB[1], NB[2], NB[3], NB[4], NB[3], NB[2], NB[1], NB[0]};
    for (int b = 0; b < 9; ++b) {
      n += (size_t)co[b] * ci[b] * 9 + co[b];
      n += (size_t)co[b] * co[b] * 9 + co[b];
      layers += 2;
    }
    n += (size_t)C * NB[0] + C;
    layers += 1;
  } else {
    for (int l = 0; l < 4; ++l) {
      int ci = l == 0 ? cin : SB[l - 1];
      n += (size_t)SB[l] * ci * 9 + SB[l] + (size_t)SB[l] * SB[l] * 9 + SB[l];
      layers += 2;
    }
    for (int l = 2; l >= 0; --l) { n += (size_t)SB[l + 1] * SB[l] * 4 + SB[l]; layers += 1; }
    for (int l = 2; l >= 0; --l) {
      n += (size_t)SB[l] * (2 * SB[l]) * 9 + SB[l] + (size_t)SB[l] * SB[l] * 9 + SB[l];
      layers += 2;
    }
    n += (size_t)C * SB[0] + C;
    layers += 1;
  }
  if (n_layers) *n_layers = layers;
  return n;
}

struct LaunchCtx { int device; int num_cus; int ksplit_max = 1, ksplit_min_chunks = 4, ksplit_gate = 4; };

template <int P, int KC, int NW, int MW, int WAVES, bool POOL, bool HEAD, bool UPF = false>
hipError_t launch_conv_k(const LaunchCtx& cx, const ConvArgs& a, hipStream_t s) {
  using C = ConvCfg<P, KC, NW, MW, WAVES, UPF>;
  const int lds = C::LDS_BYTES + a.Cout * 8 + (HEAD ? ((a.head_C * 33 * 4 + 15) / 16) * 16 : 0);
  const int total = a.N * a.tiles_x * a.tiles_y * a.nct;
  const int per_cu = std::max(1, std::min(2, (160 * 1024) / lds));
  dim3 grid((unsigned)std::min(total, cx.num_cus * per_cu));
  auto k = conv3x3_bias_relu_kernel<P, KC, NW, MW, WAVES, POOL, HEAD, UPF>;
  hipError_t st = allow_full_lds((const void*)k, cx.device);
  if (st != hipSuccess) return st;
  hipLaunchKernelGGL(k, grid, dim3(C::NT), lds, s, a);
  return hipGetLastError();
}

template <int P, bool POOL, bool HEAD, bool UPF, bool C0F = false, int NW = 1, int MW = 4, bool X8 = false, bool CAT2 = false>
hipError_t launch_ws_k(const LaunchCtx& cx, ConvArgs a, hipStream_t s) {
  using C = WsCfg<P, UPF, C0F, NW, MW, X8>;
  a.tiles_x = (a.W + C::TW - 1) / C::TW; a.tiles_y = (a.H + C::TH - 1) / C::TH; a.nct = a.Cout / C::BN;
  const int lds = C::LDS_BYTES + a.Cout * 8 + (HEAD ? ((a.head_C * 33 * 4 + 15) / 16) * 16 : 0);
  const int tiles = a.N * a.tiles_x * a.tiles_y * a.nct;
  int ks = 1;
  if (!UPF && !C0F && !HEAD && a.kpart && a.kcnt && cx.ksplit_max > 1 && tiles * cx.ksplit_gate <= cx.num_cus)
    for (int d = 2; d <= cx.ksplit_max && tiles * d <= cx.num_cus && a.nchunks / d >= cx.ksplit_min_chunks; ++d)
      if (a.nchunks % d == 0 && !(a.pair9 && (a.nchunks / d) % 2)) ks = d;
  a.ksplit = ks;
  const int total = tiles * ks;
  dim3 grid((unsigned)std::min(total, cx.num_cus));
  {
    int t = (int)grid.x;
    a.gdec[0] = t % ks; t /= ks;
    a.gdec[1] = t % a.nct; t /= a.nct;
    a.gdec[2] = t % a.tiles_x; t /= a.tiles_x;
    a.gdec[3] = t % a.tiles_y;
    a.gdec[4] = t / a.tiles_y;
  }
  auto k = conv3x3_ws_kernel<P, POOL, HEAD, UPF, C0F, NW, MW, X8, CAT2>;
  hipError_t st = allow_full_lds((const void*)k, cx.device);
  if (st != hipSuccess) return st;
  hipLaunchKernelGGL(k, grid, dim3(C::NT), lds, s, a);
  return hipGetLastError();
}

template <bool X8>
hipError_t launch_ws_x(const LaunchCtx& cx, int P, const ConvArgs& a, bool pool, bool head, bool upf, bool c0f, hipStream_t s) {
  if (P != 2 || (upf && (pool || head)) || (pool && head)) return hipErrorInvalidValue;
  if (a.Cout >= 64 && a.Cout % 64 == 0) {
    if (head || c0f) return hipErrorInvalidValue;
    if (upf) return launch_ws_k<2, false, false, true, false, 2, 2, X8>(cx, a, s);
    if (pool) return a.in1 ? hipErrorInvalidValue : launch_ws_k<2, true, false, false, false, 2, 2, X8>(cx, a, s);
    if (a.in1) return launch_ws_k<2, false, false, false, false, 2, 2, X8, true>(cx, a, s);
    return launch_ws_k<2, false, false, false, false, 2, 2, X8>(cx, a, s);
  }
  if (a.in1 && !upf) return hipErrorInvalidValue;
  if (a.Cout != 32) return hipErrorInvalidValue;
  if (c0f) return (pool && !head && !upf && a.nchunks == 2) ? launch_ws_k<2, true, false, false, true, 1, 4, X8>(cx, a, s) : hipErrorInvalidValue;
  if (upf) return launch_ws_k<2, false, false, true, false, 1, 4, X8>(cx, a, s);
  if (head) return launch_ws_k<2, false, true, false, false, 1, 4, X8>(cx, a, s);
  if (pool) return launch_ws_k<2, true, false, false, false, 1, 4, X8>(cx, a, s);
  return launch_ws_k<2, false, false, false, false, 1, 4, X8>(cx, a, s);
}

hipError_t launch_ws(const LaunchCtx& cx, int P, bool x8, const ConvArgs& a, bool pool, bool head, bool upf, bool c0f, hipStream_t s) {
  return x8 ? launch_ws_x<true>(cx, P, a, pool, head, upf, c0f, s) : launch_ws_x<false>(cx, P, a, pool, head, upf, c0f, s);
}

template <int P, int KC, int NW, int MW, int WAVES>
hipError_t launch_conv_cfg(const LaunchCtx& cx, const ConvArgs& a, bool pool, bool head, bool upf, hipStream_t s) {
  if (a.zinit) return hipErrorInvalidValue;
  if constexpr (P == 2) {
    if (pool || head || upf) return hipErrorInvalidValue;
  } else {
    if constexpr (NW == 1 && MW == 2 && KC == 16) {
      if (upf) return (pool || head) ? hipErrorInvalidValue : launch_conv_k<P, KC, NW, MW, WAVES, false, false, true>(cx, a, s);
    }
    if (upf) return hipErrorInvalidValue;
    if constexpr (NW == 1) {
      if (head) return launch_conv_k<P, KC, NW, MW, WAVES, false, true>(cx, a, s);
    }
    if constexpr (MW == 2) {
      if (pool) return launch_conv_k<P, KC, NW, MW, WAVES, true, false>(cx, a, s);
    }
    if (pool) return hipErrorInvalidValue;
  }
  return launch_conv_k<P, KC, NW, MW, WAVES, false, false>(cx, a, s);
}

hipError_t launch_conv(const LaunchCtx& cx, int P, const ConvLayer& L, int mw, const ConvArgs& a, bool head, hipStream_t s) {
#define CASE(p, kc, nw, mw_, wv) \
  if (P == p && L.KC == kc && L.NW == nw && mw == mw_ && L.WAVES == wv) return launch_conv_cfg<p, kc, nw, mw_, wv>(cx, a, L.do_pool, head, L.upf, s);
  CASE(1, 16, 1, 2, 8)
  CASE(1, 32, 2, 2, 8)
  CASE(1, 16, 2, 2, 8)
  CASE(1, 16, 4, 2, 8)
  CASE(2, 16, 2, 2, 8)
  CASE(1, 16, 2, 1, 8)
  CASE(1, 32, 2, 1, 8)
  CASE(1, 16, 4, 1, 8)
  CASE(2, 16, 2, 1, 8)
#undef CASE
  return hipErrorInvalidValue;
}

int small_grid_rows(const ConvLayer& L, int num_cus, int nb, int H, int W, bool head) {
  if (L.do_pool || head || L.upf || L.zt >= 0 || L.NW == 1 || L.MW != 2) return L.MW;
  const int tiles = nb * ((W + 31) / 32) * ((H + 15) / 16) * (L.cout / (32 * L.NW));
  return tiles < num_cus ? 1 : L.MW;
}

void choose_cfg(int P, int cin_tensor, ConvLayer& L) {
  L.MW = 2; L.WAVES = 8;
  if (P == 1) {
    if (L.cout == 32) { L.NW = 1; L.KC = 16; }
    else if (L.cout == 64) { L.NW = 2; L.KC = (cin_tensor <= 16) ? 16 : 32; }
    else { L.NW = 4; L.KC = 16; }
  } else {
    L.KC = 16;
    L.NW = (L.cout == 32) ? 1 : 2;
  }
}

struct Launcher {
  unetpp_engine* e;
  hipStream_t s;
  int rc = UNETPP_OK;
  template <class F>
  void run(const std::string& name, double flops, double bytes, F&& f) {
    if (rc) return;
    ProfRec* r = nullptr;
    auto new_event = [&]() {
      if ((size_t)e->ev_used >= e->evpool.size()) {
        hipEvent_t ev = nullptr;
        hipError_t es = hipEventCreate(&ev);
        if (es != hipSuccess) { rc = fail(e, UNETPP_E_HIP, "hipEventCreate: %s", hipGetErrorString(es)); return -1; }
        e->evpool.push_back(ev);
      }
      return e->ev_used++;
    };
    if (e->prof_on) {
      if ((size_t)e->prof_used >= e->prof.size()) e->prof.push_back(ProfRec());
      r = &e->prof[e->prof_used++];
      r->name = name; r->flops = flops; r->bytes = bytes;
      if (e->prof_prev_ev >= 0 && e->prof_prev_stream == s) {
        r->ev0 = e->prof_prev_ev;
      } else {
        r->ev0 = new_event();
        if (r->ev0 < 0) { --e->prof_used; return; }
        (void)hipEventRecord(e->evpool[r->ev0], s);
      }
    }
    hipError_t st = f();
    if (st == hipSuccess) st = hipGetLastError();
    if (r) {
      r->ev1 = new_event();
      if (r->ev1 < 0) { --e->prof_used; e->prof_prev_ev = -1; return; }
      (void)hipEventRecord(e->evpool[r->ev1], s);
      e->prof_prev_ev = r->ev1; e->prof_prev_stream = s;
    }
    if (st != hipSuccess) rc = fail(e, UNETPP_E_HIP, "launch %s: %s", name.c_str(), hipGetErrorString(st));
  }
};

struct Builder {
  unetpp_engine* e;
  size_t act = 0;
  size_t off = 0;
  int tensor(const std::string& name, int C, int lvl, bool virt = false) {
    Tensor t;
    t.name = name; t.C = C; t.lvl = lvl; t.off = act; t.virt = virt;
    const unetpp_config& c = e->cfg;
    size_t px = (size_t)e->mb * (c.max_h >> lvl) * (c.max_w >> lvl);
    if (!virt) act += align_up(px * e->P * C * sizeof(half_t), 256);
    e->tensors.push_back(t);
    return (int)e->tensors.size() - 1;
  }
  int tensor_raw(const std::string& name, size_t bytes_per_px, int lvl) {
    Tensor t;
    t.name = name; t.C = 0; t.lvl = lvl; t.off = act;
    const unetpp_config& c = e->cfg;
    size_t px = (size_t)e->mb * (c.max_h >> lvl) * (c.max_w >> lvl);
    act += align_up(px * bytes_per_px, 256);
    e->tensors.push_back(t);
    return (int)e->tensors.size() - 1;
  }
  int conv(const std::string& name, int cin_real, int in, int in2, int out, bool pool_to = false, int pool = -1, bool emit_op = true) {
    ConvLayer L;
    L.name = name; L.cin_real = cin_real; L.in = in; L.in2 = in2; L.out = out; L.pool = pool; L.do_pool = pool_to;
    L.cout = e->tensors[out].C; L.lvl = e->tensors[out].lvl;
    L.w_off = off; off += (size_t)L.cout * cin_real * 9;
    L.b_off = off; off += L.cout;
    const int c0 = e->tensors[in].C, c1 = in2 >= 0 ? e->tensors[in2].C : 0;
    choose_cfg(e->P, c0 + c1, L);
    L.nchunks = (c0 + L.KC - 1) / L.KC + c1 / L.KC;
    e->convs.push_back(L);
    Op op; op.kind = OP_CONV; op.idx = (int)e->convs.size() - 1;
    if (emit_op) e->ops.push_back(op);
    return op.idx;
  }
  void convt(const std::string& name, int in, int out) {
    ConvTLayer T;
    T.name = name; T.in = in; T.out = out; T.cin = e->tensors[in].C; T.cout = e->tensors[out].C; T.lvl = e->tensors[in].lvl;
    T.w_off = off; off += (size_t)T.cin * T.cout * 4;
    T.b_off = off; off += T.cout;
    e->convts.push_back(T);
    Op op; op.kind = OP_CONVT; op.idx = (int)e->convts.size() - 1;
    e->ops.push_back(op);
  }
  void up(int src, int dst) { Op op; op.kind = OP_UP; op.idx = src; op.out = dst; e->ops.push_back(op); }
  void ds(int k, int node) { Op op; op.kind = OP_DS; op.idx = k; op.out = node; e->ops.push_back(op); }
  void head(int in, int cx) {
    e->t_head_in = in; e->head_cx = cx;
    e->head_w_off = off; off += (size_t)e->cfg.num_classes * cx;
    e->head_b_off = off; off += e->cfg.num_classes;
    Op op; op.kind = OP_HEAD; op.out = in; e->ops.push_back(op);
  }
};

void build_nested(unetpp_engine* e, Builder& b) {
  const bool c0f = e->P == 2;
  if (!c0f) { Op cv; cv.kind = OP_CONVERT; e->ops.push_back(cv); }
  e->t_in8 = b.tensor("in8", 8, 0, c0f);
  int x[5], xa[5], pooled[4], up[4], d[4], da[4];
  for (int l = 0; l < 5; ++l) {
    char nm[32];
    snprintf(nm, sizeof nm, "x%d_0", l);
    xa[l] = b.tensor(std::string(nm) + "a", NB[l], l, c0f && l == 0);
    x[l] = b.tensor(nm, NB[l], l);
    if (l < 4) pooled[l] = b.tensor(std::string(nm) + "p", NB[l], l + 1);
    snprintf(nm, sizeof nm, "conv%d_0", l);
    const int c1 = b.conv(std::string(nm) + ".conv1", l == 0 ? 3 : NB[l - 1], l == 0 ? e->t_in8 : pooled[l - 1], -1, xa[l], false, -1,
                          !(c0f && l == 0));
    const int c2 = b.conv(std::string(nm) + ".conv2", NB[l], xa[l], -1, x[l], l < 4, l < 4 ? pooled[l] : -1);
    if (c0f && l == 0) { e->convs[c2].c0f = true; e->c0f_conv1 = c1; }
  }
  for (int l = 3; l >= 0; --l) {
    char nm[32], tn[32];
    snprintf(tn, sizeof tn, "x%d_%d", l, 4 - l);
    const int low = l == 3 ? x[4] : d[l + 1];
    const char* tl = getenv("UNETPP_TAPMM");
    const bool tapmm = e->P == 2 && l >= 1 && (9 * NB[l]) % TapmmCfg::TN == 0 && strchr(tl ? tl : "23", '0' + l) != nullptr;
    if (tapmm) {
      snprintf(nm, sizeof nm, "conv%d_%d", l, 4 - l);
      const int yt = b.tensor_raw(std::string(tn) + "y", (size_t)9 * NB[l] * 4, l + 1);
      const int zt = b.tensor_raw(std::string(tn) + "z", (size_t)NB[l] * 4, l);
      da[l] = b.tensor(std::string(tn) + "a", NB[l], l);
      d[l] = b.tensor(tn, NB[l], l);
      { Op op; op.kind = OP_TAPMM; op.idx = (int)e->convs.size(); e->ops.push_back(op); }
      { Op op; op.kind = OP_UPSUM; op.idx = (int)e->convs.size(); e->ops.push_back(op); }
      const int ci = b.conv(std::string(nm) + ".conv1", NB[l] + NB[l + 1], x[l], -1, da[l]);
      ConvLayer& L = e->convs[ci];
      L.zt = zt; L.y_t = yt; L.low_t = low;
      L.nchunks = NB[l] / L.KC;
      b.conv(std::string(nm) + ".conv2", NB[l], da[l], -1, d[l]);
      b.ds(l, d[l]);
      continue;
    }
    const bool upf = e->P == 2 || l == 0;
    if (!upf) up[l] = b.tensor(std::string(tn) + "u", NB[l + 1], l);
    da[l] = b.tensor(std::string(tn) + "a", NB[l], l);
    d[l] = b.tensor(tn, NB[l], l);
    if (!upf) b.up(low, up[l]);
    snprintf(nm, sizeof nm, "conv%d_%d", l, 4 - l);
    const int ci = b.conv(std::string(nm) + ".conv1", NB[l] + NB[l + 1], x[l], upf ? low : up[l], da[l]);
    e->convs[ci].upf = upf;
    b.conv(std::string(nm) + ".conv2", NB[l], da[l], -1, d[l]);
    if (l == 0) e->ops.back().fuse_head = true;
    else b.ds(l, d[l]);
  }
  b.head(d[0], NB[0]);
}

void build_simple(unetpp_engine* e, Builder& b) {
  Op cv; cv.kind = OP_CONVERT; e->ops.push_back(cv);
  e->t_in8 = b.tensor("in8", 8, 0);
  int enc[4], enca[4], pooled[3];
  for (int l = 0; l < 4; ++l) {
    char nm[32];
    snprintf(nm, sizeof nm, "enc%d", l + 1);
    enca[l] = b.tensor(std::string(nm) + "a", SB[l], l);
    enc[l] = b.tensor(nm, SB[l], l);
    if (l < 3) pooled[l] = b.tensor(std::string(nm) + "p", SB[l], l + 1);
    b.conv(std::string(nm) + ".0", l == 0 ? 3 : SB[l - 1], l == 0 ? e->t_in8 : pooled[l - 1], -1, enca[l]);
    b.conv(std::string(nm) + ".2", SB[l], enca[l], -1, enc[l], l < 3, l < 3 ? pooled[l] : -1);
  }
  size_t up_w[3], up_b[3], dec_w[3][2], dec_b[3][2];
  size_t off = b.off;
  for (int l = 2; l >= 0; --l) { up_w[l] = off; off += (size_t)SB[l + 1] * SB[l] * 4; up_b[l] = off; off += SB[l]; }
  for (int l = 2; l >= 0; --l) {
    dec_w[l][0] = off; off += (size_t)SB[l] * 2 * SB[l] * 9; dec_b[l][0] = off; off += SB[l];
    dec_w[l][1] = off; off += (size_t)SB[l] * SB[l] * 9; dec_b[l][1] = off; off += SB[l];
  }
  int prev = enc[3];
  for (int l = 2; l >= 0; --l) {
    char nm[32];
    snprintf(nm, sizeof nm, "up%d", l + 1);
    int u = b.tensor(std::string(nm) + "t", SB[l], l);
    b.convt(nm, prev, u);
    e->convts.back().w_off = up_w[l]; e->convts.back().b_off = up_b[l];
    snprintf(nm, sizeof nm, "dec%d", l + 1);
    int da = b.tensor(std::string(nm) + "a", SB[l], l);
    int d = b.tensor(nm, SB[l], l);
    int c1 = b.conv(std::string(nm) + ".0", 2 * SB[l], u, enc[l], da);
    e->convs[c1].w_off = dec_w[l][0]; e->convs[c1].b_off = dec_b[l][0];
    int c2 = b.conv(std::string(nm) + ".2", SB[l], da, -1, d);
    e->convs[c2].w_off = dec_w[l][1]; e->convs[c2].b_off = dec_b[l][1];
    prev = d;
  }
  b.off = off;
  b.head(prev, SB[0]);
}

}

extern "C" {

#ifndef UNETPP_SRC_HASH
#define UNETPP_SRC_HASH "unknown"
#endif
#ifdef UNETPP_WS_DBG
#define UNETPP_BUILD_TAG " +wsdbg"
#else
#define UNETPP_BUILD_TAG ""
#endif
const char* unetpp_version(void) { return "unetpp-hip 0.3.0 (gfx950) src:" UNETPP_SRC_HASH UNETPP_BUILD_TAG; }

const char* unetpp_last_error(const unetpp_engine* e) { return e ? e->err.c_str() : g_create_error.c_str(); }

size_t unetpp_weights_blob_bytes(int num_classes, int in_channels) {
  return 32 + 4 * blob_payload_floats(UNETPP_ARCH_NESTED, num_classes, in_channels);
}

size_t unetpp_weights_blob_bytes_arch(int arch, int num_classes, int in_channels) {
  if (arch != UNETPP_ARCH_NESTED && arch != UNETPP_ARCH_SIMPLE) return 0;
  return 32 + 4 * blob_payload_floats(arch, num_classes, in_channels);
}

int unetpp_create(const unetpp_config* cfg, unetpp_engine** out) {
  if (!cfg || !out) return fail(nullptr, UNETPP_E_INVALID, "null argument");
  *out = nullptr;
  if (cfg->arch != UNETPP_ARCH_NESTED && cfg->arch != UNETPP_ARCH_SIMPLE) return fail(nullptr, UNETPP_E_INVALID, "arch=%d unknown", cfg->arch);
// ... 735 lines not shown
```

Measured before the change: 3999 frames/s.

## Read conv kernel args via kernarg pointer and split out split-K kernel variant

After: 4054 frames/s (median of 6 runs). 1.4% higher.

```diff
diff --git a/unet-_amd/csrc/conv3x3_mfma.h b/unet-_amd/csrc/conv3x3_mfma.h
--- a/unet-_amd/csrc/conv3x3_mfma.h
+++ b/unet-_amd/csrc/conv3x3_mfma.h
@@ -117,6 +117,18 @@
   asm volatile("" :: "s"(touched));
 }
 
+template <class Args>
+using KernArgs = const __attribute__((address_space(4))) Args*;
+template <class Args>
+__device__ __forceinline__ KernArgs<Args> kernargs_again(KernArgs<Args> p) {
+  asm volatile("" : "+s"(p));
+  return p;
+}
+template <class Args>
+__device__ __forceinline__ KernArgs<Args> kernargs() {
+  return kernargs_again<Args>((KernArgs<Args>)__builtin_amdgcn_kernarg_segment_ptr());
+}
+
 __device__ __forceinline__ void glds16(const void* sbase, unsigned voff, unsigned lds_dst) {
   unsigned keep;
   asm volatile("s_mov_b32 %0, m0\n\ts_mov_b32 m0, %3\n\ts_nop 0\n\tglobal_load_lds_dwordx4 %1, %2\n\ts_mov_b32 m0, %0"
@@ -138,6 +150,25 @@
                  : "=&s"(keep)
                  : "v"(voff), "s"(rsrc), "s"(soff), "s"(lds_dst)
                  : "memory");
+}
+
+__device__ __forceinline__ unsigned m0_run_begin() {
+  unsigned keep;
+  asm volatile("s_mov_b32 %0, m0" : "=s"(keep) :: "memory");
+  return keep;
+}
+__device__ __forceinline__ void m0_run_end(unsigned keep) {
+  asm volatile("s_mov_b32 m0, %0" :: "s"(keep) : "memory");
+}
+__device__ __forceinline__ void glds16_run(const void* sbase, unsigned voff, unsigned lds_dst) {
+  asm volatile("s_mov_b32 m0, %2\n\ts_nop 0\n\tglobal_load_lds_dwordx4 %0, %1" :: "v"(voff), "s"(sbase), "s"(lds_dst) : "memory");
+}
+template <bool NT = false>
+__device__ __forceinline__ void blds16_run(__amdgpu_buffer_rsrc_t rsrc, unsigned voff, int soff, unsigned lds_dst) {
+  if (NT)
+    asm volatile("s_mov_b32 m0, %3\n\ts_nop 0\n\tbuffer_load_dwordx4 %0, %1, %2 offen nt lds" :: "v"(voff), "s"(rsrc), "s"(soff), "s"(lds_dst) : "memory");
+  else
+    asm volatile("s_mov_b32 m0, %3\n\ts_nop 0\n\tbuffer_load_dwordx4 %0, %1, %2 offen lds" :: "v"(voff), "s"(rsrc), "s"(soff), "s"(lds_dst) : "memory");
 }
 
 __device__ __forceinline__ void split_pack2(float v0, float v1, unsigned& wh, unsigned& wl) {
diff --git a/unet-_amd/csrc/conv3x3_ws.h b/unet-_amd/csrc/conv3x3_ws.h
--- a/unet-_amd/csrc/conv3x3_ws.h
+++ b/unet-_amd/csrc/conv3x3_ws.h
@@ -41,13 +41,19 @@
   __builtin_amdgcn_fence(__ATOMIC_ACQUIRE, "workgroup", "local");
 }
 
+template <class T>
+__device__ __forceinline__ T opaque(T v) {
+  asm volatile("" : "+s"(v));
+  return v;
+}
+
 template <int P, int ROWS, bool POOL, bool HEAD, bool X8 = false>
-__device__ __forceinline__ void ws_epilogue(const ConvArgs& a, const float16v (&acc)[ROWS], const float2* sb_lds,
+__device__ __forceinline__ void ws_epilogue(KernArgs<ConvArgs> a, const float16v (&acc)[ROWS], const float2* sb_lds,
                                             const float* head_lds, int n, int gy0, int x0, int cbase, int lane) {
-  const int H = a.H, W = a.W;
+  const int H = a->H, W = a->W;
   const int h = lane >> 5;
   const int gx = x0 + (lane & 31);
-  const int nbo = a.Cout >> 4;
+  const int nbo = a->Cout >> 4;
   float v[ROWS][16];
   float vmax = 0.f;
 #pragma unroll
@@ -61,7 +67,7 @@
     }
   }
   if (!HEAD && __builtin_amdgcn_ballot_w64(vmax > F16_MAX)) {
-    range_flag(a.status, vmax > F16_MAX, false);
+    range_flag(a->status, vmax > F16_MAX, false);
 #pragma unroll
     for (int r = 0; r < 16; ++r)
 #pragma unroll
@@ -73,9 +79,9 @@
       const int gy = gy0 + m;
       const bool ok = gy < H && gx < W;
       const size_t blk = (size_t)H * W * P * 16;
-      half_t* dst = a.out + ((size_t)n * nbo + (cbase >> 4)) * blk + ((size_t)gy * W + gx) * P * 16;
-#ifdef UNETPP_WS_DBG
-      pack_store_rows8<P, X8>(v[m], dst, blk, ok, h, (a.dbg & 262144) != 0, (a.dbg & 524288) != 0);
+      half_t* dst = a->out + ((size_t)n * nbo + (cbase >> 4)) * blk + ((size_t)gy * W + gx) * P * 16;
+#ifdef UNETPP_WS_DBG
+      pack_store_rows8<P, X8>(v[m], dst, blk, ok, h, (a->dbg & 262144) != 0, (a->dbg & 524288) != 0);
 #else
       pack_store_rows8<P, X8>(v[m], dst, blk, ok, h);
 #endif
@@ -89,14 +95,14 @@
 #pragma unroll
       for (int c = 0; c < HEAD_FUSED_MAX_CLASSES; ++c) {
         lg[c] = -INFINITY;
-        if (c < a.head_C) {
+        if (c < a->head_C) {
           float wq[16];
 #pragma unroll
           for (int q = 0; q < 4; ++q) {
             const float4 w4 = *(const float4*)(head_lds + c * 32 + 16 * (q >> 1) + 8 * h + 4 * (q & 1));
             wq[4 * q] = w4.x; wq[4 * q + 1] = w4.y; wq[4 * q + 2] = w4.z; wq[4 * q + 3] = w4.w;
           }
-          const float bc = head_lds[a.head_C * 32 + c];
+          const float bc = head_lds[a->head_C * 32 + c];
           float p0 = 0.f, p1 = 0.f;
 #pragma unroll
           for (int r = 0; r < 16; ++r) { p0 = fmaf(v[2 * m2][r], wq[r], p0); p1 = fmaf(v[2 * m2 + 1][r], wq[r], p1); }
@@ -115,30 +121,30 @@
       for (int c = 1; c < HEAD_FUSED_MAX_CLASSES; ++c)
         if (lg[c] > best) { best = lg[c]; besti = c; }
       bool is_cable = besti == 1, is_tape = besti == 2;
-      if (a.probs || a.rule) {
+      if (a->probs || a->rule) {
         float pe[HEAD_FUSED_MAX_CLASSES], sum = 0.f;
 #pragma unroll
         for (int c = 0; c < HEAD_FUSED_MAX_CLASSES; ++c) {
-          pe[c] = (c < a.head_C) ? expf(lg[c] - best) : 0.f;
+          pe[c] = (c < a->head_C) ? expf(lg[c] - best) : 0.f;
           sum += pe[c];
         }
 #pragma unroll
         for (int c = 0; c < HEAD_FUSED_MAX_CLASSES; ++c) {
           pe[c] = pe[c] / sum;
-          if (ok && a.probs && c < a.head_C) a.probs[((size_t)n * a.head_C + c) * hw + pix] = pe[c];
-        }
-        if (a.rule) apply_rule(a.rule, pe[0], pe[1], pe[2], a.t_cable, a.t_tape, a.bg_margin, a.ct_margin, is_cable, is_tape);
+          if (ok && a->probs && c < a->head_C) a->probs[((size_t)n * a->head_C + c) * hw + pix] = pe[c];
+        }
+        if (a->rule) apply_rule(a->rule, pe[0], pe[1], pe[2], a->t_cable, a->t_tape, a->bg_margin, a->ct_margin, is_cable, is_tape);
       }
       if (ok) {
-        if (a.logits) {
+        if (a->logits) {
 #pragma unroll
           for (int c = 0; c < HEAD_FUSED_MAX_CLASSES; ++c)
-            if (c < a.head_C) a.logits[((size_t)n * a.head_C + c) * hw + pix] = lg[c];
+            if (c < a->head_C) a->logits[((size_t)n * a->head_C + c) * hw + pix] = lg[c];
         }
         const size_t o = (size_t)n * hw + pix;
-        if (a.mask) a.mask[o] = (uint8_t)besti;
-        if (a.cable) a.cable[o] = is_cable;
-        if (a.tape) a.tape[o] = is_tape;
+        if (a->mask) a->mask[o] = (uint8_t)besti;
+        if (a->cable) a->cable[o] = is_cable;
+        if (a->tape) a->tape[o] = is_tape;
       }
     }
   }
@@ -157,9 +163,9 @@
       const int py = (gy0 >> 1) + m2, px = (x0 >> 1) + ((lane & 31) >> 1);
       const bool ok = ((lane & 1) == 0) && py < Hp && px < Wp;
       const size_t blk = (size_t)Hp * Wp * P * 16;
-      half_t* dst = a.pool_out + ((size_t)n * nbo + (cbase >> 4)) * blk + ((size_t)py * Wp + px) * P * 16;
-#ifdef UNETPP_WS_DBG
-      pack_store_rows8<P, X8>(pv, dst, blk, ok, h, (a.dbg & 262144) != 0);
+      half_t* dst = a->pool_out + ((size_t)n * nbo + (cbase >> 4)) * blk + ((size_t)py * Wp + px) * P * 16;
+#ifdef UNETPP_WS_DBG
+      pack_store_rows8<P, X8>(pv, dst, blk, ok, h, (a->dbg & 262144) != 0);
 #else
       pack_store_rows8<P, X8>(pv, dst, blk, ok, h);
 #endif
@@ -167,9 +173,11 @@
   }
 }
 
-template <int P, bool POOL, bool HEAD, bool UPF, bool C0F = false, int NW = 1, int MWP = 4, bool X8 = false, bool CAT2 = false>
-__global__ __launch_bounds__(512, 2) void conv3x3_ws_kernel(ConvArgs a) {
+template <int P, bool POOL, bool HEAD, bool UPF, bool C0F, int NW, int MWP, bool X8, bool CAT2, bool SPLITK>
+__device__ __forceinline__ void conv3x3_ws_body() {
   using C = WsCfg<P, UPF, C0F, NW, MWP, X8>;
+  static_assert(!SPLITK || (!UPF && !C0F && !HEAD), "split-K: plain and pooling layers only (launch_ws_k)");
+  KernArgs<ConvArgs> a = kernargs<ConvArgs>();
   static_assert(!C0F || (!UPF && !HEAD && P == 2 && NW == 1), "fused first block: exact mode, no other fusion in the loader");
   static_assert(!HEAD || NW == 1, "the fused head needs all 32 channels of x0_4 in one 32-block");
   constexpr int NT = C::NT, MW = C::MW, TH = C::TH, TW = C::TW, HALO_W = C::HALO_W;
@@ -185,20 +193,20 @@
   const int tid = threadIdx.x;
   const int lane = tid & 63;
   const int wave = __builtin_amdgcn_readfirstlane(tid >> 6);
-  const int H = a.H, W = a.W;
-  const int tiles_img = a.tiles_x * a.tiles_y;
-  const int KS = a.ksplit;
-  const int total_tiles = a.N * tiles_img * a.nct * KS;
-  const int nch0 = (a.C0 + KC - 1) / KC;
+  const int H = a->H, W = a->W;
+  const int tiles_img = a->tiles_x * a->tiles_y;
+  const int KS = SPLITK ? a->ksplit : 1;
+  const int total_tiles = a->N * tiles_img * a->nct * KS;
+  const int nch0 = (a->C0 + KC - 1) / KC;
   const unsigned lds_base = (unsigned)(unsigned long)(lds_char_t*)smem;
 
   float2* sb_lds = (float2*)(smem + C::LDS_BYTES);
-  float* head_lds = (float*)(smem + C::LDS_BYTES + a.Cout * 8);
+  float* head_lds = (float*)(smem + C::LDS_BYTES + a->Cout * 8);
   if (wave < C::NCONS) {
-    for (int i = tid; i < a.Cout; i += C::NCONS * 64) sb_lds[i] = make_float2(a.scale[i], a.bias[i]);
+    for (int i = tid; i < a->Cout; i += C::NCONS * 64) sb_lds[i] = make_float2(a->scale[i], a->bias[i]);
     if (HEAD) {
-      for (int i = tid; i < a.head_C * 32; i += C::NCONS * 64) head_lds[i] = a.head_w[i];
-      for (int i = tid; i < a.head_C; i += C::NCONS * 64) head_lds[a.head_C * 32 + i] = a.head_b[i];
+      for (int i = tid; i < a->head_C * 32; i += C::NCONS * 64) head_lds[i] = a->head_w[i];
+      for (int i = tid; i < a->head_C; i += C::NCONS * 64) head_lds[a->head_C * 32 + i] = a->head_b[i];
     }
   }
 
@@ -208,49 +216,64 @@
   const int G = (int)gridDim.x;
   const int slot = (G % 8 == 0) ? ((int)blockIdx.x % 8) * (G / 8) + (int)blockIdx.x / 8 : (int)blockIdx.x;
   int dec_ks = 0, dec_ct = 0, dec_tx = 0, dec_ty = 0, dec_n = 0, dec_t = -1;
-  const int g_ks = a.gdec[0], g_ct = a.gdec[1], g_tx = a.gdec[2], g_ty = a.gdec[3], g_n = a.gdec[4];
-  const bool small_radix = total_tiles < (1 << 22);
+  constexpr bool REREAD = HEAD;
+  auto tiles_end = [&]() {
+    if (!REREAD) return total_tiles;
+    KernArgs<ConvArgs> p = kernargs_again(a);
+    return p->N * p->tiles_x * p->tiles_y * p->nct;
+  };
+  auto tile_step = [&]() {
+    if (!REREAD) return G;
+    KernArgs<ConvArgs> p = kernargs_again(a);
+    return ((p->gdec[4] * p->tiles_y + p->gdec[3]) * p->tiles_x + p->gdec[2]) * p->nct + p->gdec[1];
+  };
   auto divmod = [&](const int u, const int d, int& q, int& r) {
     int qq, rr;
-    if (small_radix) {
+    if (opaque(tiles_end()) < (1 << 22)) {
       qq = (int)((float)u * __builtin_amdgcn_rcpf((float)d));
       rr = u - qq * d;
       const int up = rr >= d ? 1 : 0, dn = rr < 0 ? 1 : 0;
       qq += up - dn; rr += (dn - up) * d;
     } else {
-      qq = u / d; rr = u - qq * d;
+      const int dd = opaque(d);
+      qq = u / dd; rr = u - qq * dd;
     }
     q = qq; r = rr;
+  };
+  auto decode_first = [&](int t) {
+    int u = t;
+    if (SPLITK) divmod(u, KS, u, dec_ks);
+    divmod(u, a->nct, u, dec_ct);
+    divmod(u, a->tiles_x, u, dec_tx);
+    divmod(u, a->tiles_y, dec_n, dec_ty);
+  };
+  auto decode_next = [&]() {
+    KernArgs<ConvArgs> p = REREAD ? kernargs_again(a) : a;
+    const int g_ks = SPLITK ? p->gdec[0] : 0, g_ct = p->gdec[1], g_tx = p->gdec[2], g_ty = p->gdec[3], g_n = p->gdec[4];
+    dec_ks += g_ks;
+    int carry = dec_ks >= KS ? 1 : 0;
+    dec_ks -= carry ? KS : 0;
+    dec_ct += g_ct + carry;
+    carry = dec_ct >= p->nct ? 1 : 0;
+    dec_ct -= carry ? p->nct : 0;
+    dec_tx += g_tx + carry;
+    carry = dec_tx >= p->tiles_x ? 1 : 0;
+    dec_tx -= carry ? p->tiles_x : 0;
+    dec_ty += g_ty + carry;
+    carry = dec_ty >= p->tiles_y ? 1 : 0;
+    dec_ty -= carry ? p->tiles_y : 0;
+    dec_n += g_n + carry;
   };
   auto decode = [&](int t, int& n, int& y0, int& x0) {
     if (t != dec_t) {
-      if (dec_t >= 0 && t == dec_t + G) {
-        dec_ks += g_ks;
-        int carry = dec_ks >= KS ? 1 : 0;
-        dec_ks -= carry ? KS : 0;
-        dec_ct += g_ct + carry;
-        carry = dec_ct >= a.nct ? 1 : 0;
-        dec_ct -= carry ? a.nct : 0;
-        dec_tx += g_tx + carry;
-        carry = dec_tx >= a.tiles_x ? 1 : 0;
-        dec_tx -= carry ? a.tiles_x : 0;
-        dec_ty += g_ty + carry;
-        carry = dec_ty >= a.tiles_y ? 1 : 0;
-        dec_ty -= carry ? a.tiles_y : 0;
-        dec_n += g_n + carry;
-      } else {
-        int u = t;
-        divmod(u, KS, u, dec_ks);
-        divmod(u, a.nct, u, dec_ct);
-        divmod(u, a.tiles_x, u, dec_tx);
-        divmod(u, a.tiles_y, dec_n, dec_ty);
-      }
+      if (dec_t >= 0 && t == dec_t + tile_step()) decode_next();
+      else decode_first(t);
       dec_t = t;
     }
     n = dec_n; x0 = dec_tx * TW; y0 = dec_ty * TH;
   };
   if (slot >= total_tiles) return;
-  const bool handoff = C::HANDOFF && a.nchunks >= 2 && KS == 1;
+  auto handoff_on = [&]() { KernArgs<ConvArgs> p = kernargs_again(a); return C::HANDOFF && p->nchunks >= 2 && (!SPLITK || p->ksplit == 1); };
 
   typedef __attribute__((ext_vector_type(4))) float float4v;
   const int plane_id = tid - C::NCONS * 64;
@@ -262,7 +285,7 @@
     for (int i = 0; i < PATCH_LOADS; ++i) {
       const int e = plane_id + i * (C::NPROD * 64);
       int row, col, cs, idx;
-      if (a.raw_fmt == 0) {
+      if (a->raw_fmt == 0) {
         const int ch = e / (C::PATCH_H * C::PATCH_W), rem = e - ch * (C::PATCH_H * C::PATCH_W);
         row = rem / C::PATCH_W; col = rem - row * C::PATCH_W; cs = ch; idx = rem * 3 + ch;
       } else {
@@ -276,14 +299,14 @@
   auto patch_fetch = [&](int n, int y0, int x0, float (&val)[PATCH_LOADS]) {
     const size_t img = (size_t)H * W * 3;
     const __amdgpu_buffer_rsrc_t rs = __builtin_amdgcn_make_buffer_rsrc(
-        (void*)((const char*)a.raw_in + (size_t)n * img * (a.raw_fmt == 0 ? 4 : 1)), 0, (int)(img * (a.raw_fmt == 0 ? 4 : 1)), 0x00020000);
+        (void*)((const char*)a->raw_in + (size_t)n * img * (a->raw_fmt == 0 ? 4 : 1)), 0, (int)(img * (a->raw_fmt == 0 ? 4 : 1)), 0x00020000);
     bool beyond = false;
 #pragma unroll
     for (int i = 0; i < PATCH_LOADS; ++i) {
       const int gy = y0 - 2 + (pe_rc[i] >> 16), gx = x0 - 2 + ((pe_rc[i] >> 2) & 0x3fff), cs = pe_rc[i] & 3;
       const bool ok = pe_idx[i] >= 0 && gy >= 0 && gy < H && gx >= 0 && gx < W;
       float v;
-      if (a.raw_fmt == 0) {
+      if (a->raw_fmt == 0) {
         v = __builtin_bit_cast(float, __builtin_amdgcn_raw_buffer_load_b32(rs, ok ? ((cs * H + gy) * W + gx) * 4 : (int)0x80000000, 0, 0));
       } else {
         const unsigned char b8 = __builtin_amdgcn_raw_buffer_load_b8(rs, ok ? (gy * W + gx) * 3 + cs : (int)0x80000000, 0, 0);
@@ -296,7 +319,7 @@
       bool nan = false;
 #pragma unroll
       for (int i = 0; i < PATCH_LOADS; ++i) { nan |= val[i] != val[i]; val[i] = __builtin_amdgcn_fmed3f(val[i], -F16_MAX, F16_MAX); }
-      range_flag(a.status, beyond, nan);
+      range_flag(a->status, beyond, nan);
     }
   };
   auto patch_store = [&](int buf, const float (&val)[PATCH_LOADS]) {
@@ -316,7 +339,7 @@
       const int piece = (wave - C::NCONS) + it * C::NPROD;
       if (piece < 2 * C::SLAB_PIECES) {
         const int c = piece / C::SLAB_PIECES, pc = piece - c * C::SLAB_PIECES;
-        glds16((const char*)a.wpk + (size_t)c * C::SLAB_BYTES + pc * 1024, lane * 16,
+        glds16((const char*)a->wpk + (size_t)c * C::SLAB_BYTES + pc * 1024, lane * 16,
                lds_base + c * C::BUF_BYTES + C::HALO_BYTES + pc * 1024);
       }
     }
@@ -335,9 +358,9 @@
 #ifdef UNETPP_WS_DBG
 #define WS_STAMP(i) { const unsigned long long now_ = __builtin_readcyclecounter(); st_sum[i] += now_ - st_t; st_t = now_; \
                       if (ev_ptr && ev_ptr < ev_end) *ev_ptr++ = ((unsigned long long)(i) << 56) | __builtin_amdgcn_s_memrealtime(); }
-#define WS_EVLOG(role) unsigned long long* ev_ptr = (a.stamps && (a.dbg & 131072) && lane == 0 && blockIdx.x < 1024) ? a.stamps + (size_t)1024 * 32 + ((size_t)blockIdx.x * 2 + (role)) * 64 : nullptr; \
+#define WS_EVLOG(role) unsigned long long* ev_ptr = (a->stamps && (a->dbg & 131072) && lane == 0 && blockIdx.x < 1024) ? a->stamps + (size_t)1024 * 32 + ((size_t)blockIdx.x * 2 + (role)) * 64 : nullptr; \
                        unsigned long long* const ev_end = ev_ptr + 60; if (ev_ptr) *ev_ptr++ = (63ull << 56) | rt_entry;
-#define WS_STAMP_IN(i) if (a.dbg & 32768) { __builtin_amdgcn_sched_barrier(0); asm volatile("s_waitcnt lgkmcnt(0)" ::: "memory"); WS_STAMP(i) __builtin_amdgcn_sched_barrier(0); }
+#define WS_STAMP_IN(i) if (a->dbg & 32768) { __builtin_amdgcn_sched_barrier(0); asm volatile("s_waitcnt lgkmcnt(0)" ::: "memory"); WS_STAMP(i) __builtin_amdgcn_sched_barrier(0); }
 #define WS_EVT(i) { if (ev_ptr && ev_ptr < ev_end) *ev_ptr++ = ((unsigned long long)(i) << 56) | __builtin_amdgcn_s_memrealtime(); }
 #else
 #define WS_STAMP(i) {}
@@ -362,14 +385,14 @@
     half8 wa_h[2], wa_l[2];
 #pragma unroll
     for (int c = 0; c < 2; ++c) {
-      wa_h[c] = *(const half8*)(a.c1w + ((size_t)(c * 2 + 0) * 64 + lane) * 8);
-      wa_l[c] = *(const half8*)(a.c1w + ((size_t)(c * 2 + 1) * 64 + lane) * 8);
+      wa_h[c] = *(const half8*)(a->c1w + ((size_t)(c * 2 + 0) * 64 + lane) * 8);
+      wa_l[c] = *(const half8*)(a->c1w + ((size_t)(c * 2 + 1) * 64 + lane) * 8);
     }
     float sc1[2][4], bi1[2][4];
 #pragma unroll
     for (int c = 0; c < 2; ++c)
 #pragma unroll
-      for (int r = 0; r < 4; ++r) { sc1[c][r] = a.c1_scale[16 * c + 4 * kq + r]; bi1[c][r] = a.c1_bias[16 * c + 4 * kq + r]; }
+      for (int r = 0; r < 4; ++r) { sc1[c][r] = a->c1_scale[16 * c + 4 * kq + r]; bi1[c][r] = a->c1_bias[16 * c + 4 * kq + r]; }
     int koff[8];
 #pragma unroll
     for (int i = 0; i < 8; ++i) {
@@ -468,7 +491,7 @@
         };
         if (y0 >= 1 && y0 + TH < H && x0 >= 1 && x0 + TW < W) groups(std::true_type());
         else groups(std::false_type());
-        if (__builtin_amdgcn_ballot_w64(vmax > F16_MAX)) range_flag(a.status, vmax > F16_MAX, false);
+        if (__builtin_amdgcn_ballot_w64(vmax > F16_MAX)) range_flag(a->status, vmax > F16_MAX, false);
         WS_STAMP(1)
         if (have_next) patch_store(tbuf ^ 1, pv);
         WS_STAMP(2)
@@ -477,10 +500,10 @@
       }
     }
 #ifdef UNETPP_WS_DBG
-    if (a.stamps && pw == 0 && lane == 0)
-#pragma unroll
-      for (int i = 0; i < 11; ++i) a.stamps[((size_t)blockIdx.x * 2 + 1) * 16 + i] = st_sum[i];
-    if (a.stamps && pw == 0 && lane == 0) a.stamps[((size_t)blockIdx.x * 2 + 1) * 16 + 12] = __builtin_amdgcn_s_memrealtime();
+    if (a->stamps && pw == 0 && lane == 0)
+#pragma unroll
+      for (int i = 0; i < 11; ++i) a->stamps[((size_t)blockIdx.x * 2 + 1) * 16 + i] = st_sum[i];
+    if (a->stamps && pw == 0 && lane == 0) a->stamps[((size_t)blockIdx.x * 2 + 1) * 16 + 12] = __builtin_amdgcn_s_memrealtime();
 #endif
     return;
   }
@@ -489,13 +512,13 @@
     const int pw = wave - C::NCONS;
 #ifdef UNETPP_WS_DBG
     const unsigned long long rt_prod = __builtin_amdgcn_s_memrealtime();
-    { const int pr = (a.dbg >> 10) & 3; if (pr == 1) __builtin_amdgcn_s_setprio(1); else if (pr == 2) __builtin_amdgcn_s_setprio(2); else if (pr == 3) __builtin_amdgcn_s_setprio(3); }
+    { const int pr = (a->dbg >> 10) & 3; if (pr == 1) __builtin_amdgcn_s_setprio(1); else if (pr == 2) __builtin_amdgcn_s_setprio(2); else if (pr == 3) __builtin_amdgcn_s_setprio(3); }
 #endif
     constexpr unsigned OOB = 0x80000000u;
     constexpr int ITERS = C::HALO_ITERS;
     int my_u = lane / PPP;
 #ifdef UNETPP_WS_DBG
-    if (a.dbg & 16384) my_u = lane % C::U;
+    if (a->dbg & 16384) my_u = lane % C::U;
 #endif
     const int my_pl = my_u / KG, my_k8 = (my_u % KG) * 8;
     int hyx[ITERS];
@@ -503,17 +526,17 @@
     for (int it = 0; it < ITERS; ++it) {
       int hp = (pw + it * C::NPROD) * PPP + lane % PPP;
 #ifdef UNETPP_WS_DBG
-      if (a.dbg & 16384) hp = (pw + it * C::NPROD) * PPP + lane / C::U;
+      if (a->dbg & 16384) hp = (pw + it * C::NPROD) * PPP + lane / C::U;
 #endif
       const int hy = hp / HALO_W, hx = hp - hy * HALO_W;
       hyx[it] = (hp < C::NHALO) ? ((hy << 8) | hx) : -1;
     }
-    const int cb0 = a.C0 < 16 ? a.C0 : 16;
+    const int cb0 = a->C0 < 16 ? a->C0 : 16;
     const unsigned plane_bytes0 = (unsigned)H * (unsigned)W * (unsigned)(P * cb0 * 2);
-    const unsigned img_bytes0 = (unsigned)H * (unsigned)W * (unsigned)(P * a.C0 * 2);
+    const unsigned img_bytes0 = (unsigned)H * (unsigned)W * (unsigned)(P * a->C0 * 2);
     const int Hs = H >> 1, Ws = W >> 1;
     const unsigned plane_bytes1 = (unsigned)Hs * (unsigned)Ws * (unsigned)(P * 16 * 2);
-    const unsigned img_bytes1 = (unsigned)Hs * (unsigned)Ws * (unsigned)(P * a.C1 * 2);
+    const unsigned img_bytes1 = (unsigned)Hs * (unsigned)Ws * (unsigned)(P * a->C1 * 2);
     const float up_sh = Hs > 1 ? (float)(Hs - 1) / (float)(H - 1) : 0.f;
     const float up_sw = Ws > 1 ? (float)(Ws - 1) / (float)(W - 1) : 0.f;
 
@@ -521,7 +544,7 @@
 #pragma unroll
     for (int it = 0; it < ITERS; ++it) {
       const int hy = hyx[it] >> 8, hx = hyx[it] & 255;
-      const bool valid = hyx[it] >= 0 && my_k8 < a.C0;
+      const bool valid = hyx[it] >= 0 && my_k8 < a->C0;
       lane_off0[it] = valid ? (my_k8 >> 4) * (int)plane_bytes0 + ((((hy - 1) * W + (hx - 1)) * P + my_pl) * cb0 + (my_k8 & 15)) * 2 : (int)OOB;
     }
     unsigned voff0[ITERS];
@@ -533,7 +556,7 @@
     int up_st[UPR][4];
     int rd_swap = (P == 2 && !X8 && (lane & 16)) ? 32 : 0;
 #ifdef UNETPP_WS_DBG
-    if (a.dbg & 32) rd_swap = 0;
+    if (a->dbg & 32) rd_swap = 0;
 #endif
     if (UPF) {
 #pragma unroll
@@ -561,16 +584,20 @@
         for (int it = 0; it < ITERS; ++it) {
           const int hy = hyx[it] >> 8, hx = hyx[it] & 255;
           const int gy = y0 + hy - 1, gx = x0 + hx - 1;
-          const bool ok = hyx[it] >= 0 && gy >= 0 && gy < H && gx >= 0 && gx < W;
+          const bool ok = (hyx[it] | gy | gx) >= 0 && gy < H && gx < W;
           const unsigned pix = (unsigned)((gy * W + gx) * P + my_pl);
-          voff0[it] = (ok && my_k8 < a.C0) ? (unsigned)(my_k8 >> 4) * plane_bytes0 + (pix * cb0 + (my_k8 & 15)) * 2u : OOB;
-        }
-      }
-      rsrc0 = __builtin_amdgcn_make_buffer_rsrc((void*)(a.in0 + (size_t)n * H * W * P * a.C0), 0, (int)img_bytes0, 0x00020000);
-      if (CAT2)
-        rsrc1 = __builtin_amdgcn_make_buffer_rsrc((void*)(a.in1 + (size_t)n * H * W * P * a.C1), 0, (int)((unsigned)H * (unsigned)W * (unsigned)(P * a.C1 * 2)), 0x00020000);
+          voff0[it] = (ok && my_k8 < a->C0) ? (unsigned)(my_k8 >> 4) * plane_bytes0 + (pix * cb0 + (my_k8 & 15)) * 2u : OOB;
+        }
+      }
+      KernArgs<ConvArgs> at = REREAD ? kernargs_again(a) : a;
+      const unsigned img0 = REREAD ? (unsigned)H * (unsigned)W * (unsigned)(P * at->C0 * 2) : img_bytes0;
+      rsrc0 = __builtin_amdgcn_make_buffer_rsrc((void*)(at->in0 + (size_t)n * (img0 >> 1)), 0, (int)img0, 0x00020000);
+      if (CAT2) {
+        const unsigned img_bytes_cat = (unsigned)H * (unsigned)W * (unsigned)(P * a->C1 * 2);
+        rsrc1 = __builtin_amdgcn_make_buffer_rsrc((void*)(a->in1 + (size_t)n * (img_bytes_cat >> 1)), 0, (int)img_bytes_cat, 0x00020000);
+      }
       if (UPF) {
-        rsrc1 = __builtin_amdgcn_make_buffer_rsrc((void*)(a.in1 + (size_t)n * Hs * Ws * P * a.C1), 0, (int)img_bytes1, 0x00020000);
+        rsrc1 = __builtin_amdgcn_make_buffer_rsrc((void*)(a->in1 + (size_t)n * (img_bytes1 >> 1)), 0, (int)img_bytes1, 0x00020000);
         const int ybase = (int)(up_sh * (float)max(y0 - 1, 0)), xbase = (int)(up_sw * (float)max(x0 - 1, 0));
         constexpr int PXP = 1024 / C::LS_REC, PARTS = C::LS_REC / 16;
 #pragma unroll
@@ -628,7 +655,7 @@
 #pragma unroll
         for (int k = 0; k < 4; ++k) {
 #ifdef UNETPP_WS_DBG
-          if (a.dbg & 512) { hq[r][k] = (u32x2){0x3c003c00u, 0x3c003c00u}; lq[r][k] = (u32x2){0u, 0u}; continue; }
+          if (a->dbg & 512) { hq[r][k] = (u32x2){0x3c003c00u, 0x3c003c00u}; lq[r][k] = (u32x2){0u, 0u}; continue; }
 #endif
           hq[r][k] = *(const u32x2*)(ls + off[k]);
           if (P == 2) lq[r][k] = *(const u32x2*)(ls + (off[k] ^ 32));
@@ -668,7 +695,7 @@
         }
         WS_STAMP_IN(9)
 #ifdef UNETPP_WS_DBG
-        if (a.dbg & 64) { if (v[0][0] == 12345.f && v[3][3] == 7.f && v[1][2] == 3.f && v[2][1] == 9.f) a.status[1] = 1; continue; }
+        if (a->dbg & 64) { if (v[0][0] == 12345.f && v[3][3] == 7.f && v[1][2] == 3.f && v[2][1] == 9.f) a->status[1] = 1; continue; }
 #endif
         if (up_st[r][0] >= 0) {
 #pragma unroll
@@ -697,8 +724,7 @@
     };
 
     const int stg_base = 2 * C::BUF_BYTES + 2 * C::LS_BYTES + 2 * C::PATCH_BYTES;
-    int hn = 0, hy0 = 0, hx0 = 0, hct = 0;
-    bool have_handoff = false;
+    int hn = -1, hty = 0, htx = 0, hct = 0;
     auto handoff_epilogue = [&]() {
       const char* st = smem + stg_base + pw * C::STG_WAVE + lane * 16;
       float16v pair[2];
@@ -710,104 +736,114 @@
           const f32x4 v4 = *(const f32x4*)(st + (i * 4 + q) * 1024);
           pair[i][4 * q] = v4[0]; pair[i][4 * q + 1] = v4[1]; pair[i][4 * q + 2] = v4[2]; pair[i][4 * q + 3] = v4[3];
         }
-      const int gy0 = hy0 + pw * MW + (MW == 4 ? 2 : 0);
+      const int gy0 = hty * TH + pw * MW + (MW == 4 ? 2 : 0);
       const int cbase = hct * BN + (MW == 4 ? 0 : 32);
-      ws_epilogue<P, 2, POOL, HEAD, X8>(a, pair, sb_lds, head_lds, hn, gy0, hx0, cbase, lane);
+      ws_epilogue<P, 2, POOL, HEAD, X8>(kernargs_again(a), pair, sb_lds, head_lds, hn, gy0, htx * TW, cbase, lane);
     };
     int g = 0;
-    const bool slabs_stay = a.nchunks == 2 && a.nct == 1 && KS == 1;
-    const int chunks_per_share = KS == 1 ? a.nchunks : a.nchunks / KS;
 #ifdef UNETPP_WS_DBG
     st_t = __builtin_readcyclecounter();
 #endif
     WS_EVT(51)
-    for (int tile = slot; tile < total_tiles; tile += G) {
-      int n, y0, x0;
-      decode(tile, n, y0, x0);
+    decode_first(slot);
+    for (int tile = slot; tile < tiles_end(); tile += tile_step(), decode_next()) {
+      const int n = dec_n, y0 = dec_ty * TH, x0 = dec_tx * TW;
       WS_EVT(52)
-      const char* wsrc = (const char*)a.wpk + (size_t)dec_ct * a.nchunks * C::SLAB_BYTES;
-      const int tile_ct = dec_ct;
-      const int c_begin = dec_ks * chunks_per_share, c_end = c_begin + chunks_per_share;
+      const int handoff_c = opaque((handoff_on() && hn >= 0) ? 1 : -1);
+      KernArgs<ConvArgs> at = REREAD ? kernargs_again(a) : a;
+      const int nchunks = at->nchunks;
+      const bool slabs_stay = nchunks == 2 && at->nct == 1 && KS == 1;
+      const int chunks_per_share = KS == 1 ? nchunks : nchunks / KS;
+      const char* wsrc = (const char*)at->wpk + (size_t)dec_ct * nchunks * C::SLAB_BYTES;
+      const int c_begin = dec_ks * chunks_per_share, c_end = c_begin + opaque(chunks_per_share);
       setup_tile(n, y0, x0);
       WS_STAMP(7)
       for (int c = c_begin; c < c_end; ++c, ++g) {
         const int buf = (g & 1) * C::BUF_BYTES;
-#ifdef UNETPP_WS_DBG
-        if (!(a.dbg & 2))
+        const unsigned dst0 = opaque(lds_base + buf + pw * 1024);
+        const unsigned m0_keep = m0_run_begin();
+#ifdef UNETPP_WS_DBG
+        if (!(a->dbg & 2))
 #endif
         if (c < nch0) {
+          const int soff = c * (int)plane_bytes0;
 #pragma unroll
           for (int it = 0; it < ITERS; ++it) {
             const int piece = pw + it * C::NPROD;
-            if (C::HALO_PIECES % C::NPROD == 0 || piece < C::HALO_PIECES)
-              blds16<true>(rsrc0, voff0[it], c * (int)plane_bytes0, lds_base + buf + piece * 1024);
+            if (it + 1 < ITERS || C::HALO_PIECES % C::NPROD == 0 || piece < C::HALO_PIECES)
+              blds16_run<true>(rsrc0, voff0[it], soff, dst0 + it * (C::NPROD * 1024));
           }
         } else if (CAT2) {
+          const int soff = (c - nch0) * (int)plane_bytes0;
 #pragma unroll
           for (int it = 0; it < ITERS; ++it) {
             const int piece = pw + it * C::NPROD;
-            if (C::HALO_PIECES % C::NPROD == 0 || piece < C::HALO_PIECES)
-              blds16<true>(rsrc1, voff0[it], (c - nch0) * (int)plane_bytes0, lds_base + buf + piece * 1024);
+            if (it + 1 < ITERS || C::HALO_PIECES % C::NPROD == 0 || piece < C::HALO_PIECES)
+              blds16_run<true>(rsrc1, voff0[it], soff, dst0 + it * (C::NPROD * 1024));
           }
         }
 #ifdef UNETPP_WS_DBG
-        if (!(a.dbg & 8))
-#endif
-        if (!(slabs_stay && g >= 2))
-#pragma unroll
-        for (int it = 0; it < C::SLAB_ITERS; ++it) {
-          const int piece = pw + it * C::NPROD;
-          if (C::SLAB_PIECES % C::NPROD == 0 || piece < C::SLAB_PIECES)
-            glds16(wsrc + (size_t)c * C::SLAB_BYTES + piece * 1024, lane * 16, lds_base + buf + C::HALO_BYTES + piece * 1024);
-        }
-        if (!UPF) { WS_STAMP(0) }
+        if (!(a->dbg & 8))
+#endif
+        if (!(slabs_stay && g >= 2)) {
+          const char* wchunk = opaque(wsrc + (size_t)c * C::SLAB_BYTES + pw * 1024);
+#pragma unroll
+          for (int it = 0; it < C::SLAB_ITERS; ++it) {
+            const int piece = pw + it * C::NPROD;
+            if (it + 1 < C::SLAB_ITERS || C::SLAB_PIECES % C::NPROD == 0 || piece < C::SLAB_PIECES)
+              glds16_run(wchunk + it * (C::NPROD * 1024), lane * 16, dst0 + C::HALO_BYTES + it * (C::NPROD * 1024));
+          }
+        }
+        if (!UPF) { m0_run_end(m0_keep); WS_STAMP(0) }
         if (UPF) {
 #ifdef UNETPP_WS_DBG
-          if (!(a.dbg & 2))
-#endif
-          if (c + 1 < a.nchunks && c + 1 >= nch0) {
+          if (!(a->dbg & 2))
+#endif
+          if (c + 1 < nchunks && c + 1 >= nch0) {
+            const int soffL = (c + 1 - nch0) * (int)plane_bytes1;
+            const unsigned dstL = opaque(lds_base + 2 * C::BUF_BYTES + ((c + 1) & 1) * C::LS_BYTES + pw * 1024);
 #pragma unroll
             for (int it = 0; it < LSR; ++it) {
               const int piece = pw + it * C::NPROD;
-              if (C::LS_PIECES % C::NPROD == 0 || piece < C::LS_PIECES)
-                blds16(rsrc1, voffL[it], (c + 1 - nch0) * (int)plane_bytes1,
-                       lds_base + 2 * C::BUF_BYTES + ((c + 1) & 1) * C::LS_BYTES + piece * 1024);
+              if (it + 1 < LSR || C::LS_PIECES % C::NPROD == 0 || piece < C::LS_PIECES)
+                blds16_run(rsrc1, voffL[it], soffL, dstL + it * (C::NPROD * 1024));
             }
           }
+          m0_run_end(m0_keep);
           if (c >= nch0) { WS_STAMP(3) } else { WS_STAMP(0) }
 #ifdef UNETPP_WS_DBG
-          if (!(a.dbg & 1))
+          if (!(a->dbg & 1))
 #endif
           if (c >= nch0) up_rounds(c, buf);
           if (c >= nch0) { WS_STAMP(4) } else { WS_STAMP(0) }
         }
 #ifdef UNETPP_WS_DBG
-        if (!(a.dbg & 128))
-#endif
-        if (handoff && c == 1 && have_handoff) handoff_epilogue();
+        if (!(a->dbg & 128))
+#endif
+        if (c == handoff_c) handoff_epilogue();
         asm volatile("s_waitcnt vmcnt(0)" ::: "memory");
         if (UPF && c >= nch0) { WS_STAMP(5) } else { WS_STAMP(1) }
         lds_barrier();
         if (UPF && c >= nch0) { WS_STAMP(6) } else { WS_STAMP(2) }
       }
-      hn = n; hy0 = y0; hx0 = x0; hct = tile_ct; have_handoff = true;
-    }
-    if (handoff) {
+      hn = dec_n; hty = dec_ty; htx = dec_tx; hct = dec_ct;
+    }
+    if (handoff_on()) {
       lds_barrier();
-      if (have_handoff) handoff_epilogue();
-    }
-#ifdef UNETPP_WS_DBG
-    if (a.stamps && pw == 0 && lane == 0)
-#pragma unroll
-      for (int i = 0; i < 11; ++i) a.stamps[((size_t)blockIdx.x * 2 + 1) * 16 + i] = st_sum[i];
-    if (a.stamps && pw == 0 && lane == 0) a.stamps[((size_t)blockIdx.x * 2 + 1) * 16 + 12] = __builtin_amdgcn_s_memrealtime();
+      if (hn >= 0) handoff_epilogue();
+    }
+#ifdef UNETPP_WS_DBG
+    if (a->stamps && pw == 0 && lane == 0)
+#pragma unroll
+      for (int i = 0; i < 11; ++i) a->stamps[((size_t)blockIdx.x * 2 + 1) * 16 + i] = st_sum[i];
+    if (a->stamps && pw == 0 && lane == 0) a->stamps[((size_t)blockIdx.x * 2 + 1) * 16 + 12] = __builtin_amdgcn_s_memrealtime();
 #endif
     return;
   }
 
   const int cw = wave;
 #ifdef UNETPP_WS_DBG
-  { const int pr = (a.dbg >> 12) & 3; if (pr == 1) __builtin_amdgcn_s_setprio(1); else if (pr == 2) __builtin_amdgcn_s_setprio(2); else if (pr == 3) __builtin_amdgcn_s_setprio(3); }
+  { const int pr = (a->dbg >> 12) & 3; if (pr == 1) __builtin_amdgcn_s_setprio(1); else if (pr == 2) __builtin_amdgcn_s_setprio(2); else if (pr == 3) __builtin_amdgcn_s_setprio(3); }
 #endif
   int a_off[MW + 2][3];
 #pragma unroll
@@ -883,20 +919,21 @@
   if (cw != 0) ev_ptr = nullptr;
   if (ev_ptr) *ev_ptr++ = (62ull << 56) | rt_begin;
 #endif
-  for (int tile = slot; tile < total_tiles; tile += G) {
-    int n, y0, x0;
-    decode(tile, n, y0, x0);
+  decode_first(slot);
+  for (int tile = slot; tile < tiles_end(); tile += tile_step(), decode_next()) {
+    const int n = dec_n, y0 = dec_ty * TH, x0 = dec_tx * TW;
     const int ct = dec_ct, ks = dec_ks;
-    const int c_begin = ks * (a.nchunks / KS), c_end = c_begin + a.nchunks / KS;
+    const bool handoff = handoff_on();
+    const int c_begin = ks * (a->nchunks / KS), c_end = c_begin + a->nchunks / KS;
 #pragma unroll
     for (int m = 0; m < MW; ++m)
 #pragma unroll
       for (int j = 0; j < NW; ++j) {
-        if (a.zinit && ks == 0) {
+        if (a->zinit && ks == 0) {
           typedef __attribute__((ext_vector_type(4))) float f32x4;
           const int gy = y0 + cw * MW + m, gx = x0 + (lane & 31);
           const bool in = gy < H && gx < W;
-          const float* zp = a.zinit + (((size_t)n * (a.Cout >> 5) + ((ct * BN + j * 32) >> 5)) * ((size_t)H * W) + (size_t)gy * W + gx) * 32 + 8 * (lane >> 5);
+          const float* zp = a->zinit + (((size_t)n * (a->Cout >> 5) + ((ct * BN + j * 32) >> 5)) * ((size_t)H * W) + (size_t)gy * W + gx) * 32 + 8 * (lane >> 5);
 #pragma unroll
           for (int q = 0; q < 4; ++q) {
             f32x4 z4 = {0.f, 0.f, 0.f, 0.f};
@@ -906,7 +943,7 @@
           }
         }
       }
-    const bool from_zero = a.zinit == nullptr || ks != 0;
+    const bool from_zero = a->zinit == nullptr || ks != 0;
     int4v x9[MW];
     if (X8) {
 #pragma unroll
@@ -919,7 +956,7 @@
       const char* halo = smem + (g & 1) * C::BUF_BYTES;
       const char* slab = halo + C::HALO_BYTES;
 #ifdef UNETPP_WS_DBG
-      if (a.dbg & 16) continue;
+      if (a->dbg & 16) continue;
 #endif
       if constexpr (X8) {
         constexpr int R = MW + 2;
@@ -950,7 +987,7 @@
         };
         auto main_step = [&](const BM& b, const half8 (&hf)[R], int dy, bool first) {
 #ifdef UNETPP_WS_DBG
-          if (a.dbg & 4) return;
+          if (a->dbg & 4) return;
 #endif
           const float16v zero = {0.f, 0.f, 0.f, 0.f, 0.f, 0.f, 0.f, 0.f, 0.f, 0.f, 0.f, 0.f, 0.f, 0.f, 0.f, 0.f};
 #pragma unroll
@@ -961,7 +998,7 @@
         };
         auto cross_step = [&](const BX& b, const int8v (&x)[R], int r0) {
 #ifdef UNETPP_WS_DBG
-          if (a.dbg & (4 | 65536)) return;
+          if (a->dbg & (4 | 65536)) return;
 #endif
 #pragma unroll
           for (int m = 0; m < MW; ++m)
@@ -1026,7 +1063,7 @@
         __builtin_amdgcn_sched_barrier(0);
         cross_step(bx1, xa, 0);
         __builtin_amdgcn_sched_barrier(0);
-        if (!(a.pair9 && ((c - c_begin) & 1) == 0)) {
+        if (!(a->pair9 && ((c - c_begin) & 1) == 0)) {
           int8v xq[R];
 #pragma unroll
           for (int m = 0; m < MW; ++m) xq[m] = __builtin_shufflevector(x9[m], cur[m], 0, 1, 2, 3, 4, 5, 6, 7);
@@ -1058,7 +1095,7 @@
           if (dx < 2) load_a_part(fan, halo, dx + 1, 2 * dy, 2 * dy + 2);
           __builtin_amdgcn_sched_barrier(0);
 #ifdef UNETPP_WS_DBG
-          if (!(a.dbg & 4))
+          if (!(a->dbg & 4))
 #endif
           {
             if (step == 0 && c == c_begin && from_zero) run_mfma_first(fa, fb);
@@ -1070,14 +1107,14 @@
       WS_STAMP(1)
     }
 #ifdef UNETPP_WS_DBG
-    if (a.dbg & 256) { if (acc[0][0][0] == 12345.f && acc[MW - 1][NW - 1][5] == 7.f) a.status[1] = 1; continue; }
+    if (a->dbg & 256) { if (acc[0][0][0] == 12345.f && acc[MW - 1][NW - 1][5] == 7.f) a->status[1] = 1; continue; }
 #endif
     if (KS > 1) {
       typedef __attribute__((ext_vector_type(4))) float f32x4;
       const int tile_id = tile / KS;
       const int ntile = total_tiles / KS;
       constexpr int WAVE_BYTES = MW * NW * 16 * 64 * 4;
-      const __amdgpu_buffer_rsrc_t prs = __builtin_amdgcn_make_buffer_rsrc((void*)a.kpart, 0, KS * ntile * C::NCONS * WAVE_BYTES, 0x00020000);
+      const __amdgpu_buffer_rsrc_t prs = __builtin_amdgcn_make_buffer_rsrc((void*)a->kpart, 0, KS * ntile * C::NCONS * WAVE_BYTES, 0x00020000);
       const int mine = ((ks * ntile + tile_id) * C::NCONS + cw) * WAVE_BYTES + lane * 16;
 #pragma unroll
       for (int m = 0; m < MW; ++m)
@@ -1089,11 +1126,11 @@
                                                    prs, mine + ((m * NW + j) * 4 + q) * 1024, 0, 16 );
       asm volatile("s_waitcnt vmcnt(0)" ::: "memory");
       unsigned old = 0;
-      if (lane == 0) old = __hip_atomic_fetch_add(a.kcnt + tile_id * C::NCONS + cw, 1u, __ATOMIC_RELAXED, __HIP_MEMORY_SCOPE_AGENT);
+      if (lane == 0) old = __hip_atomic_fetch_add(a->kcnt + tile_id * C::NCONS + cw, 1u, __ATOMIC_RELAXED, __HIP_MEMORY_SCOPE_AGENT);
       old = __builtin_amdgcn_readfirstlane(old);
       if (old != (unsigned)(KS - 1)) { WS_STAMP(2) continue; }
       __builtin_amdgcn_fence(__ATOMIC_ACQUIRE, "wavefront");
-      if (lane == 0) __hip_atomic_store(a.kcnt + tile_id * C::NCONS + cw, 0u, __ATOMIC_RELAXED, __HIP_MEMORY_SCOPE_AGENT);
+      if (lane == 0) __hip_atomic_store(a->kcnt + tile_id * C::NCONS + cw, 0u, __ATOMIC_RELAXED, __HIP_MEMORY_SCOPE_AGENT);
       constexpr int HALF = MW * NW * 2;
       auto fetch = [&](f32x4 (&pv)[HALF], int u) {
         const int src = (((u >> 1) * ntile + tile_id) * C::NCONS + cw) * WAVE_BYTES + lane * 16 + (u & 1) * HALF * 1024;
@@ -1139,23 +1176,32 @@
             }
         } else {
           const float16v pair[2] = {acc[2 * m2][j], acc[2 * m2 + 1][j]};
-          ws_epilogue<P, 2, POOL, HEAD, X8>(a, pair, sb_lds, head_lds, n, y0 + cw * MW + 2 * m2, x0, ct * BN + j * 32, lane);
+          ws_epilogue<P, 2, POOL, HEAD, X8>(kernargs_again(a), pair, sb_lds, head_lds, n, y0 + cw * MW + 2 * m2, x0, ct * BN + j * 32, lane);
         }
       }
     WS_STAMP(2)
   }
-  if (handoff) lds_barrier();
-#ifdef UNETPP_WS_DBG
-  if (a.stamps && cw == 0 && lane == 0)
-#pragma unroll
-    for (int i = 0; i < 4; ++i) a.stamps[((size_t)blockIdx.x * 2) * 16 + i] = st_sum[i];
-  if (a.stamps && cw == 0 && lane == 0) {
-    a.stamps[((size_t)blockIdx.x * 2) * 16 + 4] = rt_begin;
-    a.stamps[((size_t)blockIdx.x * 2) * 16 + 6] = rt_entry;
-    a.stamps[((size_t)blockIdx.x * 2) * 16 + 5] = __builtin_amdgcn_s_memrealtime();
+  if (handoff_on()) lds_barrier();
+#ifdef UNETPP_WS_DBG
+  if (a->stamps && cw == 0 && lane == 0)
+#pragma unroll
+    for (int i = 0; i < 4; ++i) a->stamps[((size_t)blockIdx.x * 2) * 16 + i] = st_sum[i];
+  if (a->stamps && cw == 0 && lane == 0) {
+    a->stamps[((size_t)blockIdx.x * 2) * 16 + 4] = rt_begin;
+    a->stamps[((size_t)blockIdx.x * 2) * 16 + 6] = rt_entry;
+    a->stamps[((size_t)blockIdx.x * 2) * 16 + 5] = __builtin_amdgcn_s_memrealtime();
   }
 #endif
 }
 #undef WS_STAMP
 
+template <int P, bool POOL, bool HEAD, bool UPF, bool C0F = false, int NW = 1, int MWP = 4, bool X8 = false, bool CAT2 = false>
+__global__ __launch_bounds__(512, 2) void conv3x3_ws_kernel(ConvArgs) {
+  conv3x3_ws_body<P, POOL, HEAD, UPF, C0F, NW, MWP, X8, CAT2, false>();
 }
+template <int P, bool POOL, int NW = 1, int MWP = 4, bool X8 = false, bool CAT2 = false>
+__global__ __launch_bounds__(512, 2) void conv3x3_ws_splitk_kernel(ConvArgs) {
+  conv3x3_ws_body<P, POOL, false, false, false, NW, MWP, X8, CAT2, true>();
+}
+
+}
diff --git a/unet-_amd/csrc/unetpp_abi.hip b/unet-_amd/csrc/unetpp_abi.hip
--- a/unet-_amd/csrc/unetpp_abi.hip
+++ b/unet-_amd/csrc/unetpp_abi.hip
@@ -229,7 +229,10 @@
     a.gdec[3] = t % a.tiles_y;
     a.gdec[4] = t / a.tiles_y;
   }
-  auto k = conv3x3_ws_kernel<P, POOL, HEAD, UPF, C0F, NW, MW, X8, CAT2>;
+  void (*k)(ConvArgs) = conv3x3_ws_kernel<P, POOL, HEAD, UPF, C0F, NW, MW, X8, CAT2>;
+  if constexpr (!UPF && !C0F && !HEAD) {
+    if (ks > 1) k = conv3x3_ws_splitk_kernel<P, POOL, NW, MW, X8, CAT2>;
+  }
   hipError_t st = allow_full_lds((const void*)k, cx.device);
   if (st != hipSuccess) return st;
   hipLaunchKernelGGL(k, grid, dim3(C::NT), lds, s, a);
```
